# Healthcare-Robotics/mr-gan

Hardware: AMD Instinct MI355X
Metric: GAN train steps/sec (labeled+unlabeled+G) at batch 4096 (higher is better)
Workload: dtype bf16; 1 GPU; BASELINE configs[1]: synthetic N=65536 x D=512, K=6, batch 4096 per GPU, labeled 100/class; one step = D sub-step (3B rows) + G sub-step (2B rows) + both Adam updates; global_batch=4096, rows_per_gpu=4096, parallelism=single, batch_statistics=n/a, launch=hipGraph replay

## Files before the change

include/mrgan_debug.h:

```cpp
#ifndef MRGAN_DEBUG_H
#define MRGAN_DEBUG_H

#include "mrgan_abi.h"

#ifdef __cplusplus
extern "C" {
#endif

int mrgan_debug_noise(mrgan_handle* h, uint32_t site, uint32_t seg, uint32_t step, uint32_t row0, int rows, int cols,
                      float* out_dev, mrgan_stream stream);
int mrgan_debug_tr_probe(uint16_t* out1024_dev, mrgan_stream stream);
int mrgan_debug_ablate(mrgan_handle* h, int bits);
int mrgan_debug_buffer(mrgan_handle* h, int kind, int l, void** ptr_dev, int* rows_per_seg, int* ld, int* elem_size);
int mrgan_debug_gemm_time(int op, int m, int n, int k, int nbatch, int splits, int reps, int ablate, int kc_cfg, float* avg_us);

typedef struct mrgan_debug_gemm_desc {
    int32_t dtype, op, m, n, k, nbatch, splits;
    int32_t kchunk;
    int32_t kc_cfg;
    int32_t tune_bits;
    int32_t seg_stride, seg_rows;
    const void* a; int64_t a_bs, a_si, a_sk;
    const void* b; int64_t b_bs, b_sk, b_sj;
    int32_t act, n_valid;
    const float* bias;
    void* out; int64_t out_bs; int32_t ldo;
    float sigma; uint32_t site, seg0; int32_t seg_step; uint32_t iter_step, row0;
    uint32_t iter;
    uint64_t seed;
    uint16_t* mask; int64_t mask_bs; int32_t ldm;
    const void* h; int64_t h_bs; int32_t ldh;
    int32_t cs_mode; float* cs1; float* cs2; int32_t ldcs;
    const float* bn_mu; const float* bn_rstd;
    float* slab; int64_t slab_stride;
    void* q8; int64_t q8_bs; int32_t ldq8;
    void* q8t; int64_t q8t_bs; int32_t ldq8t;
    const void* slot_a; const void* slot_b; void* slot_o;
    int32_t gauss;
} mrgan_debug_gemm_desc;
typedef struct mrgan_debug_fold { const float* src; float* dst; int64_t stride; int32_t nsrc, n, ngroups; } mrgan_debug_fold;
int mrgan_debug_gemm_launch(const mrgan_debug_gemm_desc* d, int count, int grouped, const mrgan_debug_fold* fold,
                            char* kname, int kname_len, mrgan_stream stream);

int mrgan_debug_gemm_fp8(int m, int n, int k, const float* a_dev, const float* b_dev, const float* bias_dev, int act, float scale_a,
                         float scale_b, float* out_dev, int reps, float* avg_us, int kc_cfg, mrgan_stream stream);

int mrgan_debug_quant8(const void* src, int64_t src_bs, int ld, int rows, int cols, int nb, int prow, void* dst, int64_t dst_bs, int ldd,
                       void* dstt, int64_t dstt_bs, int lddt, void* slot_dev, int fmt, mrgan_stream stream);
int mrgan_debug_fp8_update_scales(void* slots_dev, int n, mrgan_stream stream);

#ifdef __cplusplus
}
#endif
#endif
```

mr_gan_amd/csrc/engine_debug.hip:

```cpp
#include "engine_internal.h"

namespace mrgan {
int launch_tr_probe(unsigned short* out, hipStream_t s);
}

namespace {

template <typename T>
__global__ void to_f32_kernel(const T* src, long lds, float* dst, long ldd, int rows, int cols) {
    const int c = blockIdx.x * 64 + (threadIdx.x & 63), r = blockIdx.y * 4 + (threadIdx.x >> 6);
    if (r >= rows || c >= cols) return;
    dst[(long)r * ldd + c] = Elem<T>::to_f32(src[(long)r * lds + c]);
}

}

extern "C" {

int mrgan_debug_noise(mrgan_handle* h, uint32_t site, uint32_t seg, uint32_t step, uint32_t row0, int rows, int cols, float* out,
                      mrgan_stream stream) {
    if (!h || !out) return fail(-1, "null argument");
    if (h->gauss && (row0 & 1u)) return fail(-1, "debug_noise: a true-Gaussian handle draws row pairs, row0 must be even");
    CHK(launch_noise_debug(h->gauss, h->cfg.seed, site, seg, step, row0, rows, cols, out, (hipStream_t)stream));
    return 0;
}

int mrgan_debug_ablate(mrgan_handle* h, int bits) {
    if (!h) return fail(-1, "null handle");
    if (h->graph_exec) { hipGraphExecDestroy(h->graph_exec); h->graph_exec = nullptr; h->graph_ready = false; }
    h->ablate = bits;
    return 0;
}

int mrgan_debug_buffer(mrgan_handle* h, int kind, int l, void** ptr, int* rows_per_seg, int* ld, int* elem_size) {
    if (!h || !ptr || l < 0 || l > 4) return fail(-1, "debug_buffer: bad argument");
    switch (kind) {
        case 0: *ptr = selected(h, h->xin[l]); *ld = h->d[l].Kp; break;
        case 1: *ptr = selected(h, h->dpre[l]); *ld = h->d[l].Np; break;
        case 2: *ptr = selected(h, h->feat); *ld = h->Fp; break;
        default: return fail(-1, "debug_buffer: unknown kind");
    }
    *rows_per_seg = h->S; *elem_size = h->es;
    return 0;
}

int mrgan_debug_gemm_time(int op, int m, int n, int k, int nbatch, int splits, int reps, int ablate, int kc_cfg, float* avg_us) {
    if ((n % 64) || (k % 64) || !avg_us) return fail(-1, "debug_gemm_time: bad argument");
    const size_t rows = (size_t)m * nbatch;
    const bool is_dx = op == 1 || op >= 5;
    const int a_cols = is_dx ? n : k, o_cols = is_dx ? k : n;
    if (op < 0 || op > 8) return fail(-1, "debug_gemm_time: bad op");
    if (!kc_cfg_supported(kc_cfg)) return fail(-1, "debug_gemm_time: unsupported forward / dX tile config %d", kc_cfg);
    __bf16 *ta = nullptr, *tb = nullptr, *to = nullptr;
    uint16_t* mask = nullptr; float* slabs = nullptr; float* bias = nullptr; DevState* st = nullptr;
    HIPCHK(hipMalloc((void**)&ta, rows * std::max(a_cols, n) * 2));
    HIPCHK(hipMalloc((void**)&tb, (size_t)std::max((size_t)k, rows) * n * 2));
    HIPCHK(hipMalloc((void**)&to, rows * std::max(o_cols, n) * 2));
    HIPCHK(hipMalloc((void**)&mask, (rows / 32 + 4) * std::max(n, k) * 4));
    HIPCHK(hipMalloc((void**)&bias, (size_t)std::max(n, k) * 4));
    HIPCHK(hipMalloc((void**)&st, sizeof(DevState) * 2));
    HIPCHK(hipMemset(ta, 0x3c, rows * std::max(a_cols, n) * 2));
    HIPCHK(hipMemset(tb, 0x3c, (size_t)std::max((size_t)k, rows) * n * 2));
    HIPCHK(hipMemset(mask, 0x55, (rows / 32 + 4) * std::max(n, k) * 4));
    HIPCHK(hipMemset(bias, 0, (size_t)std::max(n, k) * 4));
    HIPCHK(hipMemset(st, 0, sizeof(DevState) * 2));
    GemmArgs g;
    int epi;
    if (op == 0 || op == 3 || op == 4) {
        epi = EPI_FWD; g = gemm_fwd_args(m, k, n, nbatch, ta, (long)m * k, k, tb, k, true);
        g.e.act = ACT_RELU; g.e.n_valid = n; g.e.bias = bias; g.e.ldo = n; g.e.out_bs = (long)m * n;
        g.e.sigma = op == 0 ? 0.5f : 0.f; g.e.site = 1;
        if (op != 4) { g.e.mask = mask; g.e.ldm = n; g.e.mask_bs = (long)(m / 32 + 1) * n * 2; }
    } else if (is_dx) {
        epi = EPI_DX; g = gemm_dx_args(m, k, n, nbatch, ta, (long)m * n, n, tb, n);
        g.e.act = op == 1 ? ACT_RELU : op == 5 ? ACT_SOFTPLUS : ACT_LINEAR; g.e.n_valid = k; g.e.ldo = k; g.e.out_bs = (long)m * k;
        if (op == 1) { g.e.mask = mask; g.e.ldm = k; g.e.mask_bs = (long)(m / 32 + 1) * k * 2; }
        if (op == 5 || op == 6) { g.e.h = ta; g.e.ldh = k; g.e.h_bs = (long)m * k; }
        if (op >= 5 && op <= 7) {
            HIPCHK(hipMalloc((void**)&slabs, (size_t)2 * (rows / 64 + 1) * k * 4));
            g.e.cs_mode = op == 6 ? CS_SUM_XHAT : CS_SUM; g.e.cs1 = slabs; g.e.cs2 = slabs + (size_t)(rows / 64 + 1) * k; g.e.ldcs = k;
            g.e.bn_mu = bias; g.e.bn_rstd = bias;
        }
    } else {
        epi = EPI_SLAB; splits = std::max(1, splits);
        HIPCHK(hipMalloc((void**)&slabs, (size_t)splits * k * n * 4));
        g = gemm_dw_args(k, n, m * nbatch, splits, gemm_dw_kchunk(m * nbatch, splits), 0, 0, ta, k, tb, n, false, slabs);
    }
    g.e.st = st; g.e.out = to; g.e.ablate = ablate; g.e.tune_kc_cfg = kc_cfg; g.e.seed = 1;
#ifdef MRGAN_STAMPS
    unsigned long long* stamps = nullptr;
    if (op != 2) {
        HIPCHK(hipMalloc((void**)&stamps, 4096 * 12 * sizeof(unsigned long long)));
        HIPCHK(hipMemset(stamps, 0, 4096 * 12 * sizeof(unsigned long long)));
        g.e.slab = (float*)stamps;
    }
#endif
    hipEvent_t e0, e1;
    HIPCHK(hipEventCreate(&e0)); HIPCHK(hipEventCreate(&e1));
    int r = 0;
    for (int i = 0; i < 3 && !r; ++i) r = launch_gemm_bf16(epi, g, 0);
    HIPCHK(hipDeviceSynchronize());
    HIPCHK(hipEventRecord(e0, 0));
    for (int i = 0; i < reps && !r; ++i) r = launch_gemm_bf16(epi, g, 0);
    HIPCHK(hipEventRecord(e1, 0));
    HIPCHK(hipEventSynchronize(e1));
    float ms = 0.f;
    HIPCHK(hipEventElapsedTime(&ms, e0, e1));
    *avg_us = 1e3f * ms / (float)reps;
#ifdef MRGAN_STAMPS
    if (stamps) {
        std::vector<unsigned long long> hs(4096 * 12);
        hipMemcpy(hs.data(), stamps, hs.size() * 8, hipMemcpyDeviceToHost);
        double tot[10] = {0, 0, 0, 0, 0, 0, 0, 0, 0, 0}; int nb = 0;
        for (int b = 0; b < 4096; ++b) if (hs[b * 12 + 2]) { ++nb; for (int i = 0; i < 10; ++i) tot[i] += (double)hs[b * 12 + i]; }
        if (nb) fprintf(stderr, "  stamps (kcycles per block, %d blocks): setup %.1f | fill %.1f | mainloop %.1f | barrier %.1f | epilogue %.1f (math+staging %.1f, barrier %.1f, copy-out %.1f, column sums %.1f) | tail-barrier %.1f\n",
                        nb, tot[0] / nb / 1e3, tot[1] / nb / 1e3, tot[2] / nb / 1e3, tot[3] / nb / 1e3, tot[4] / nb / 1e3, tot[6] / nb / 1e3, tot[7] / nb / 1e3, tot[8] / nb / 1e3,
                        tot[9] / nb / 1e3, tot[5] / nb / 1e3);
        hipFree(stamps);
    }
#endif
    hipEventDestroy(e0); hipEventDestroy(e1);
    hipFree(ta); hipFree(tb); hipFree(to); hipFree(mask); hipFree(bias); hipFree(st);
    if (slabs) hipFree(slabs);
    if (r) return fail(r, "debug_gemm_time: launch failed (%d)", r);
    return 0;
}

int mrgan_debug_gemm_fp8(int m, int n, int k, const float* a, const float* b, const float* bias, int act, float scale_a, float scale_b,
                         float* out, int reps, float* avg_us, int kc_cfg, mrgan_stream stream) {
    if ((n % 64) || (k % 128) || !a || !b) return fail(-1, "debug_gemm_fp8: n %% 64 == 0 and k %% 128 == 0 are required");
    hipStream_t s = (hipStream_t)stream;
    unsigned char *ta = nullptr, *tb = nullptr;
    __bf16* to = nullptr;
    HIPCHK(hipMalloc((void**)&ta, (size_t)m * k));
    HIPCHK(hipMalloc((void**)&tb, (size_t)n * k));
    HIPCHK(hipMalloc((void**)&to, (size_t)m * n * 2));
    CHK(launch_to_fp8(a, k, ta, k, m, k, m, k, scale_a, 0, s));
    CHK(launch_to_fp8(b, n, tb, k, k, n, k, n, scale_b, 1, s));
    GemmArgs g = gemm_fwd_args(m, k, n, 1, ta, 0, k, tb, k, true);
    g.e.act = act; g.e.n_valid = n; g.e.bias = bias; g.e.out = to; g.e.ldo = n; g.e.acc_scale = 1.0f / (scale_a * scale_b);
    g.e.tune_kc_cfg = kc_cfg;
#ifdef MRGAN_STAMPS
    unsigned long long* stamps = nullptr;
    HIPCHK(hipMalloc((void**)&stamps, 4096 * 4 * sizeof(unsigned long long)));
    g.e.cs2 = (float*)stamps;
#endif
    int r = launch_gemm_fp8(EPI_FWD, g, s);
#ifdef MRGAN_STAMPS
    HIPCHK(hipMemsetAsync(stamps, 0, 4096 * 4 * sizeof(unsigned long long), s));
#endif
    if (!r && reps > 0 && avg_us) {
        hipEvent_t e0, e1;
        HIPCHK(hipEventCreate(&e0)); HIPCHK(hipEventCreate(&e1));
        HIPCHK(hipStreamSynchronize(s));
        HIPCHK(hipEventRecord(e0, s));
        for (int i = 0; i < reps && !r; ++i) r = launch_gemm_fp8(EPI_FWD, g, s);
        HIPCHK(hipEventRecord(e1, s));
        HIPCHK(hipEventSynchronize(e1));
        float ms = 0.f;
        HIPCHK(hipEventElapsedTime(&ms, e0, e1));
        *avg_us = 1e3f * ms / (float)reps;
        hipEventDestroy(e0); hipEventDestroy(e1);
    }
    if (!r && out) hipLaunchKernelGGL(to_f32_kernel<__bf16>, grid2d(m, n), dim3(256), 0, s, (const __bf16*)to, (long)n, out, (long)n, m, n);
    hipStreamSynchronize(s);
#ifdef MRGAN_STAMPS
    {
        std::vector<unsigned long long> hs(4096 * 4);
        hipMemcpy(hs.data(), stamps, hs.size() * 8, hipMemcpyDeviceToHost);
        double cyc = 0, wait = 0, rt = 0, tiles = 0; int nb = 0;
        for (int b = 0; b < 4096; ++b) if (hs[b * 4 + 3]) { cyc += hs[b * 4]; wait += hs[b * 4 + 1]; rt += hs[b * 4 + 2]; tiles += hs[b * 4 + 3]; ++nb; }
        if (nb) fprintf(stderr, "[stamps] fp8 %dx%dx%d: blocks %d, tiles/block %.1f, k-loop cycles/tile %.0f (wait+barrier %.0f = %.1f %%), per k-tile %.0f, clock %.3f GHz\n",
                        m, n, k, nb, tiles / nb, cyc / tiles, wait / tiles, 100.0 * wait / cyc, cyc / tiles / (k / 128), cyc / rt * 0.1);
        hipFree(stamps);
    }
#endif
    hipFree(ta); hipFree(tb); hipFree(to);
    if (r) return fail(r, "debug_gemm_fp8: launch failed (%d)", r);
    return 0;
}

int mrgan_debug_tr_probe(uint16_t* out, mrgan_stream stream) {
    if (!out) return fail(-1, "null argument");
    CHK(launch_tr_probe(out, (hipStream_t)stream));
    return 0;
}

static int debug_gemm_args(const mrgan_debug_gemm_desc& d, const DevState* st, GemmArgs& g, int& epi) {
    const bool bf = d.dtype == MRGAN_BF16, f8 = d.dtype == MRGAN_FP8;
    if (!bf && !f8 && d.dtype != MRGAN_F32) return fail(-1, "debug_gemm_launch: dtype must be fp32, bf16 or fp8");
    if (d.op < 0 || d.op > 2) return fail(-1, "debug_gemm_launch: op must be 0, 1 or 2");
    if (!kc_cfg_supported(d.kc_cfg)) return fail(-1, "debug_gemm_launch: kc_cfg %d is not a block tile", d.kc_cfg);
    if (d.m < 1 || d.n < 1 || d.k < 1 || d.nbatch < 1 || d.splits < 1 || !d.a || !d.b) return fail(-1, "debug_gemm_launch: empty problem");
    if (d.n % 64) return fail(-1, "debug_gemm_launch: n must be a multiple of 64");
    epi = d.op == 0 ? EPI_FWD : d.op == 1 ? EPI_DX : EPI_SLAB;
    if (epi == EPI_FWD) g = gemm_fwd_args(d.m, d.k, d.n, d.nbatch, d.a, d.a_bs, d.a_si, d.b, d.b_sj, true);
    else if (epi == EPI_DX) g = gemm_dx_args(d.m, d.n, d.k, d.nbatch, d.a, d.a_bs, d.a_si, d.b, d.b_sj);
    else if (f8) g = gemm_dw_args(d.m, d.n, d.k, 1, d.k, 0, 0, d.a, d.a_si, d.b, d.b_sj, true, d.slab);
    else g = gemm_dw_args(d.m, d.n, d.k, 1, d.k, 0, 0, d.a, d.a_sk, d.b, d.b_sk, false, d.slab);
    g.nbatch = d.nbatch; g.splits = d.splits;
    if (d.kchunk > 0) g.kchunk = d.kchunk;
    if (d.seg_stride > 0) { g.seg_stride = d.seg_stride; g.seg_rows = d.seg_rows; }
    g.a_bs = d.a_bs; g.a_si = d.a_si; g.a_sk = d.a_sk;
    g.b_bs = d.b_bs; g.b_sk = d.b_sk; g.b_sj = d.b_sj;
    Epi& e = g.e;
    e.act = d.act; e.n_valid = d.n_valid; e.bias = d.bias;
    e.out = d.out; e.out_bs = d.out_bs; e.ldo = d.ldo;
    e.sigma = d.sigma; e.site = d.site; e.seg0 = d.seg0; e.seg_step = d.seg_step; e.iter_step = d.iter_step; e.row0 = d.row0; e.seed = d.seed;
    e.mask = d.mask; e.mask_bs = d.mask_bs; e.ldm = d.ldm;
    e.h = d.h; e.h_bs = d.h_bs; e.ldh = d.ldh;
    e.cs_mode = d.cs_mode; e.cs1 = d.cs1; e.cs2 = d.cs2; e.ldcs = d.ldcs; e.bn_mu = d.bn_mu; e.bn_rstd = d.bn_rstd;
    e.slab = d.slab; e.slab_stride = d.slab_stride;
    e.st = st; e.acc_scale = 1.f; e.tune_kc_cfg = d.kc_cfg; e.tune_bits = d.tune_bits;
    e.gauss = d.gauss;
    if (f8) {
        e.q8 = d.q8; e.q8_bs = d.q8_bs; e.ldq8 = d.ldq8; e.q8t = d.q8t; e.q8t_bs = d.q8t_bs; e.ldq8t = d.ldq8t;
        e.qa = (const Fp8Slot*)d.slot_a; e.qb = (const Fp8Slot*)d.slot_b; e.qo = (Fp8Slot*)d.slot_o;
        if (epi == EPI_SLAB ? d.ldo < d.n : (d.out && (d.ldo < d.n || (d.ldo % 8)))) return fail(-1, "debug_gemm_launch: fp8 product needs ldo >= n (bf16: a multiple of 8)");
        if ((d.a_si % 16) || (d.b_sj % 16) || (d.a_bs % 16) || (d.b_bs % 16)) return fail(-1, "debug_gemm_launch: fp8 row and batch pitches must be multiples of 16 bytes");
        if (d.q8 && (d.q8_bs % 16)) return fail(-1, "debug_gemm_launch: q8_bs must be a multiple of 16");
        if (d.q8 && d.ldq8 < d.n) return fail(-1, "debug_gemm_launch: ldq8 >= n");
        if (d.q8t && (d.q8t_bs < 0 || d.ldq8t < (d.nbatch - 1) * d.q8t_bs + round_up(d.m, 16))) return fail(-1, "debug_gemm_launch: ldq8t must hold nbatch batches of round_up(m, 16) bytes");
    }
    if (epi == EPI_SLAB && !f8) {
        const int bk = bf ? 64 : 16;
        if (!d.slab || d.ldo < d.n) return fail(-1, "debug_gemm_launch: weight gradient needs slab and ldo >= n");
        if ((g.kchunk % bk) || (g.seg_stride % bk)) return fail(-1, "debug_gemm_launch: kchunk and seg_stride must be multiples of %d", bk);
        if (bf && ((d.a_sk % 8) || (d.b_sk % 8) || d.a_sk < round_up(d.m, 8))) return fail(-1, "debug_gemm_launch: bf16 row pitches must be multiples of 8");
    } else if (epi != EPI_SLAB) {
        if ((!f8 && !d.out) || (d.out && d.ldo < d.n) || d.n_valid < 0 || d.n_valid > d.n) return fail(-1, "debug_gemm_launch: needs out, ldo >= n and n_valid <= n");
        if (bf && ((d.ldo % 8) || (d.a_si % 8) || (d.b_sj % 8))) return fail(-1, "debug_gemm_launch: bf16 row pitches must be multiples of 8");
        if (d.cs_mode != CS_NONE && (!d.cs1 || d.ldcs < d.n || (d.cs_mode != CS_SUM && !d.cs2))) return fail(-1, "debug_gemm_launch: column sums need cs1 / cs2 and ldcs >= n");
        if (d.cs_mode == CS_SUM_XHAT && (epi != EPI_DX || !d.bn_mu || !d.bn_rstd || !d.h)) return fail(-1, "debug_gemm_launch: xhat sums need bn_mu, bn_rstd and h on a dX product");
        if (epi == EPI_DX && d.act == ACT_SOFTPLUS && !d.h) return fail(-1, "debug_gemm_launch: the softplus derivative needs h");
        if (epi == EPI_DX && d.act == ACT_RELU && !d.mask) return fail(-1, "debug_gemm_launch: the relu derivative needs mask");
        if (d.h && (d.ldh < d.n || (bf && (d.ldh % 8)))) return fail(-1, "debug_gemm_launch: ldh");
        if (d.mask && d.ldm < d.n) return fail(-1, "debug_gemm_launch: ldm >= n");
    }
    return 0;
}

int mrgan_debug_gemm_launch(const mrgan_debug_gemm_desc* d, int count, int grouped, const mrgan_debug_fold* fold,
                            char* kname, int kname_len, mrgan_stream stream) {
    if (!d || count < 1) return fail(-1, "null argument");
    if (kname && kname_len > 0) kname[0] = 0;
    hipStream_t s = (hipStream_t)stream;
    DevState* st = nullptr;
    DevState hst[2];
    memset(hst, 0, sizeof hst);
    hst[0].iter = hst[1].iter = d[0].iter;
    HIPCHK(hipMalloc((void**)&st, sizeof hst));
    hipError_t he = hipMemcpy(st, hst, sizeof hst, hipMemcpyHostToDevice);
    const char* name = "";
    int r = he == hipSuccess ? 0 : fail(-10, "hipMemcpy failed: %s", hipGetErrorString(he));
    if (!r && !grouped) {
        GemmArgs g;
        int epi = 0;
        if (count != 1) r = fail(-1, "debug_gemm_launch: one product per plain launch");
        if (!r) r = debug_gemm_args(d[0], st, g, epi);
        if (!r) {
            r = d[0].dtype == MRGAN_FP8    ? launch_gemm_fp8(epi, g, s, &name)
                : d[0].dtype == MRGAN_BF16 ? launch_gemm_bf16(epi, g, s, &name)
                                           : launch_gemm_f32(epi, g, s, &name);
            if (r) fail(r, "debug_gemm_launch: launch refused (%d)", r);
        }
    } else if (!r) {
        GemmArgs gs[KS_GROUP_MAX];
        for (int i = 0; i < count && i < KS_GROUP_MAX && !r; ++i) {
            int epi = 0;
            r = debug_gemm_args(d[i], st, gs[i], epi);
            if (!r && (epi != EPI_SLAB || d[i].dtype != MRGAN_BF16)) r = fail(-1, "debug_gemm_launch: grouped launches are bf16 weight gradients");
        }
        FoldJob fj;
        memset(&fj, 0, sizeof fj);
        if (!r && fold) {
            if (!fold->src || !fold->dst || fold->nsrc < 1 || fold->n < 1 || fold->ngroups < 1 || fold->stride < fold->n)
                r = fail(-1, "debug_gemm_launch: fold");
            fj.src = fold->src; fj.dst = fold->dst; fj.stride = fold->stride; fj.nsrc = fold->nsrc; fj.n = fold->n; fj.ngroups = fold->ngroups;
        }
        if (!r) {
            r = launch_gemm_bf16_dw_group(gs, count, s, &name, fold ? &fj : nullptr);
            if (r < 0) fail(r, "debug_gemm_launch: grouped launch failed (%d)", r);
        }
    }
    he = hipStreamSynchronize(s);
    hipFree(st);
    if (!r && he != hipSuccess) return fail(-10, "debug_gemm_launch: %s", hipGetErrorString(he));
    if (!r && kname && kname_len > 0) snprintf(kname, (size_t)kname_len, "%s", name);
    return r;
}

int mrgan_debug_quant8(const void* src, int64_t src_bs, int ld, int rows, int cols, int nb, int prow, void* dst, int64_t dst_bs, int ldd,
                       void* dstt, int64_t dstt_bs, int lddt, void* slot, int fmt, mrgan_stream stream) {
    if (!src || rows < 0 || rows > prow || cols < 1 || cols > ld || (fmt != FP8_E4M3 && fmt != FP8_E5M2)) return fail(-1, "debug_quant8: bad argument");
    if ((dst && ldd < cols) || (dstt && (dstt_bs < 0 || lddt < (int64_t)(nb - 1) * dstt_bs + prow))) return fail(-1, "debug_quant8: ldd >= cols, lddt >= nb batches of prow bytes");
    Quant8Args a;
    memset(&a, 0, sizeof a);
    a.src = (const __bf16*)src; a.src_bs = src_bs; a.ld = ld; a.rows = rows; a.cols = cols; a.nb = nb; a.prow = prow;
    a.dst = (unsigned char*)dst; a.dst_bs = dst_bs; a.ldd = ldd;
    a.dstt = (unsigned char*)dstt; a.dstt_bs = dstt_bs; a.lddt = lddt;
    a.slot = (Fp8Slot*)slot; a.fmt = fmt;
    hipStream_t s = (hipStream_t)stream;
    const int r = launch_quant8(a, s);
    if (r) return fail(r, "debug_quant8: launch refused (%d)", r);
    HIPCHK(hipStreamSynchronize(s));
    return 0;
}

int mrgan_debug_fp8_update_scales(void* slots, int n, mrgan_stream stream) {
    if (!slots || n < 1) return fail(-1, "debug_fp8_update_scales: bad argument");
    hipStream_t s = (hipStream_t)stream;
    CHK(launch_fp8_update_scales((Fp8Slot*)slots, n, s));
    HIPCHK(hipStreamSynchronize(s));
    return 0;
}

}
```

mr_gan_amd/csrc/gemm.h:

```cpp
#pragma once
#include <string.h>

#include <algorithm>

#include "common.h"

namespace mrgan {

enum { EPI_FWD = 0, EPI_DX = 1, EPI_SLAB = 2 };
enum { VAR_ACT_MASK = 3, VAR_NOISE = 4, VAR_MASK = 8, VAR_GAUSS = 16, VAR_DYN = 64 };


struct Epi {
    int act;
    int n_valid;
    const float* bias;
    void* out; long out_bs; int ldo;
    float sigma; uint32_t site; uint32_t seg0;
    int seg_step; uint32_t iter_step;
    uint32_t row0;
    uint64_t seed;
    int gauss;
    uint16_t* mask; long mask_bs; int ldm;
    const void* h; long h_bs; int ldh;
    int cs_mode; float* cs1; float* cs2; int ldcs;
    const float* bn_mu; const float* bn_rstd;
    float* slab; long slab_stride;
    const DevState* st;
    int ablate;
    float acc_scale;
    const Fp8Slot* qa; const Fp8Slot* qb;
    Fp8Slot* qo;
    void* q8; long q8_bs; int ldq8;
    void* q8t; long q8t_bs; int ldq8t;
    int tune_kc_cfg;
    int tune_bits;
    long model_stride;
    int segs;
    uint32_t model_mul;
};

struct GemmArgs {
    int M, N, K;
    int nbatch, splits;
    int kchunk;
    int tiles_m;
    int seg_stride, seg_rows;
    const void* A; long a_bs, a_si, a_sk;
    const void* B; long b_bs, b_sk, b_sj;
    Epi e;
};

__device__ __forceinline__ int batch_model(const Epi& e, int batch) { return (int)(((uint32_t)batch * e.model_mul) >> 16); }
__device__ __forceinline__ int batch_segment(const Epi& e, int batch, int model) { return batch - model * e.segs; }
template <typename P>
__device__ __forceinline__ P* model_ptr(P* p, const Epi& e, int model) { return (P*)((char*)p + (long)model * e.model_stride); }
template <typename P>
__device__ __forceinline__ const P* model_ptr(const P* p, const Epi& e, int model) { return (const P*)((const char*)p + (long)model * e.model_stride); }

__device__ __forceinline__ uint32_t relu_mask_bit(const uint16_t* mask, int ldm, int row, int col) {
    const int rr = row & 31;
    const uint32_t w = mask[((long)(row >> 5) * ldm + col) * 2 + ((rr >> 2) & 1)];
    return (w >> ((rr & 3) | ((rr >> 3) << 2))) & 1u;
}

template <int MR, int NR>
struct EpiPrefetch {
    float bias[NR];
    float mu[NR], rstd[NR];
    uint32_t mbits[MR][NR];
    uint32_t iter;
};

template <int VAR>
__device__ __host__ __forceinline__ bool dx_needs_h(const Epi& e) {
    if constexpr ((VAR & VAR_DYN) != 0) return e.h && (e.act == ACT_SOFTPLUS || e.cs_mode == CS_SUM_XHAT);
    else if constexpr ((VAR & VAR_ACT_MASK) == ACT_SOFTPLUS) return true;
    else if constexpr ((VAR & VAR_ACT_MASK) == ACT_LINEAR) return e.cs_mode == CS_SUM_XHAT;
    else return false;
}

template <typename T, int EPI, int MR, int NR, int VAR>
__device__ __forceinline__ void epilogue_prefetch(EpiPrefetch<MR, NR>& pf, const GemmArgs& g, int batch , int model,
                                                  int row_blk, int col_blk, int wm, int wn, int lane) {
    const Epi& e = g.e;
    const int lc = lane & 31, lh = lane >> 5;
    const int act = (VAR & 64) ? e.act : (VAR & 3);
    pf.iter = 0u;
    if constexpr (EPI == EPI_FWD && ((VAR & VAR_DYN) || (VAR & VAR_NOISE))) { if (e.st) pf.iter = e.st->iter; }
#pragma unroll
    for (int ni = 0; ni < NR; ++ni) {
        const int col = col_blk + (wn * NR + ni) * 32 + lc;
        pf.bias[ni] = 0.f; pf.mu[ni] = 0.f; pf.rstd[ni] = 0.f;
        if constexpr (EPI == EPI_FWD) { if (col < e.n_valid && e.bias) pf.bias[ni] = model_ptr(e.bias, e, model)[col]; }
        if constexpr (EPI == EPI_DX) {
            if (e.cs_mode == CS_SUM_XHAT) {
                const bool cok = col < e.n_valid && col < g.N;
                const int cc = cok ? col : 0;
                const float m = e.bn_mu[cc], r = e.bn_rstd[cc];
                pf.mu[ni] = cok ? m : 0.f; pf.rstd[ni] = cok ? r : 0.f;
            }
        }
#pragma unroll
        for (int mi = 0; mi < MR; ++mi) {
            pf.mbits[mi][ni] = 0;
            if constexpr (EPI == EPI_DX) {
                const int rsub = row_blk + (wm * MR + mi) * 32;
                if (act == ACT_RELU && e.mask && col < g.N && rsub < g.M)
                    pf.mbits[mi][ni] = (model_ptr(e.mask, e, model) + (long)batch * e.mask_bs)[((long)(rsub >> 5) * e.ldm + col) * 2 + lh];
            }
        }
    }
}

template <typename T, int EPI, int MR, int NR, int WM, bool STAGED = false, int VAR = VAR_DYN, int Q8 = -1>
__device__ __forceinline__ void epilogue(f32x16 (&acc)[MR][NR], const GemmArgs& g, int batch , int model, int split,
                                         int tile_m, int row_blk, int col_blk, int wm, int wn, int lane,
                                         float* lds ,
                                         int bn , T* tile = nullptr,
                                         const EpiPrefetch<MR, NR>* pf = nullptr,
                                         const T* htile = nullptr ,
                                         unsigned long long* est = nullptr ) {
#ifdef MRGAN_STAMPS
#define EPI_STAMP(i) do { if (est) { const unsigned long long n_ = __builtin_amdgcn_s_memtime(); est[i] += n_ - est[4]; est[4] = n_; } } while (0)
    if (est) est[4] = __builtin_amdgcn_s_memtime();
#else
#define EPI_STAMP(i)
#endif
    const Epi& e = g.e;
    const int lc = lane & 31, lh = lane >> 5;
    const int M = g.M;
    if (e.ablate & 2) { if (acc[0][0][0] == 12345.678f) ((float*)e.out)[0] = 1.f; return; }

    if constexpr (EPI == EPI_SLAB) {
        float* dst = model_ptr(e.slab, e, model) + (long)(batch * g.splits + split) * e.slab_stride;
#pragma unroll
        for (int mi = 0; mi < MR; ++mi)
#pragma unroll
            for (int ni = 0; ni < NR; ++ni) {
                const int col = col_blk + (wn * NR + ni) * 32 + lc;
#pragma unroll
                for (int r = 0; r < 16; ++r) {
                    const int row = row_blk + (wm * MR + mi) * 32 + acc_row(r, lh);
                    if (row < M && col < g.N) dst[(long)row * e.ldo + col] = acc[mi][ni][r];
                }
            }
        return;
    } else {
        constexpr bool DYN = (VAR & VAR_DYN) != 0;
        const int act = DYN ? e.act : (VAR & VAR_ACT_MASK);
        constexpr bool fast_math = sizeof(T) == 2;
        T* out = (T*)model_ptr(e.out, e, model) + (long)batch * e.out_bs;
        constexpr bool MASKED = !DYN && (EPI == EPI_DX || (VAR & VAR_MASK));
        uint16_t* mask = nullptr;
        if constexpr (MASKED) mask = model_ptr(e.mask, e, model) + (long)batch * e.mask_bs;
        else if (DYN && e.mask) mask = model_ptr(e.mask, e, model) + (long)batch * e.mask_bs;
        const T* hprev = e.h ? (const T*)model_ptr(e.h, e, model) + (long)batch * e.h_bs : nullptr;
        float* const cs1p = model_ptr(e.cs1, e, model);
        float* const cs2p = model_ptr(e.cs2, e, model);
        const bool noisy = EPI == EPI_FWD && (DYN ? e.sigma > 0.f : (VAR & VAR_NOISE) != 0);
        constexpr bool GAUSS = (VAR & VAR_GAUSS) != 0;
        uint32_t rowhash[MR];
        i32x4 hfrag = {0, 0, 0, 0};
        const float sigs = GAUSS ? e.sigma : e.sigma * NOISE_SCALE;
        if constexpr (EPI == EPI_FWD) {
            if (noisy) {
                const uint32_t nkey = noise_key(e.seed + (uint64_t)model, e.site * 256u + e.seg0 + (uint32_t)(batch * e.seg_step),
                                                (pf ? pf->iter : (e.st ? e.st->iter : 0u)) + (uint32_t)batch * e.iter_step);
                if constexpr (!GAUSS) hfrag = hadamard_frag(lane);
#pragma unroll
                for (int mi = 0; mi < MR; ++mi) {
                    if constexpr (GAUSS) rowhash[mi] = gauss_pairhash(nkey, e.row0 + (uint32_t)(row_blk + (wm * MR + mi) * 32), lane);
                    else rowhash[mi] = noise_rowhash(nkey, e.row0 + (uint32_t)(row_blk + (wm * MR + mi) * 32 + lc));
                }
            }
        }

        float q8_scale = 1.f, q8_amax = 0.f;
        float q8_cs[MR][NR];
        if constexpr (Q8 >= 0) {
            q8_scale = e.qo->scale;
#pragma unroll
            for (int mi = 0; mi < MR; ++mi)
#pragma unroll
                for (int ni = 0; ni < NR; ++ni) q8_cs[mi][ni] = 0.f;
        }
        float keep[MR][NR][16];
#pragma unroll
        for (int ni = 0; ni < NR; ++ni) {
            const int col = col_blk + (wn * NR + ni) * 32 + lc;
            const bool colvalid = col < e.n_valid;
            const bool colin = col < g.N;
            float bias = 0.f;
            if constexpr (EPI == EPI_FWD) {
                if (pf) bias = pf->bias[ni];
                else if (colvalid && e.bias) bias = model_ptr(e.bias, e, model)[col];
            }
            const float sig = (noisy && colvalid) ? sigs : 0.f;
#pragma unroll
            for (int mi = 0; mi < MR; ++mi) {
                const int rsub = row_blk + (wm * MR + mi) * 32;
                const long mword = ((long)(rsub >> 5) * e.ldm + col) * 2 + lh;
                uint32_t mbits = 0;
                if constexpr (EPI == EPI_DX) {
                    if (pf) mbits = pf->mbits[mi][ni];
                    else if (act == ACT_RELU && colin && rsub < M) mbits = mask[mword];
                }
                i32x16 nzs = {0, 0, 0, 0, 0, 0, 0, 0, 0, 0, 0, 0, 0, 0, 0, 0};
                f32x16 nzg = {0.f, 0.f, 0.f, 0.f, 0.f, 0.f, 0.f, 0.f, 0.f, 0.f, 0.f, 0.f, 0.f, 0.f, 0.f, 0.f};
                if constexpr (EPI == EPI_FWD) {
                    if constexpr (GAUSS) { if (noisy) nzg = gauss_block(rowhash[mi], (uint32_t)col, lane); }
                    else if (noisy) nzs = noise_block(rowhash[mi], (uint32_t)col >> 5, lane, hfrag);
                }
#pragma unroll
                for (int q = 0; q < 4; ++q) {
                    const int r4 = rsub + 4 * lh + 8 * q;
                    float o4[4];
#pragma unroll
                    for (int j = 0; j < 4; ++j) {
                        const int r = 4 * q + j, row = r4 + j;
                        float v = acc[mi][ni][r];
                        float& o = o4[j];
                        if constexpr (EPI == EPI_FWD) {
                            v += bias;
                            if (act == ACT_RELU) {
                                v = fmaxf(v, 0.f);
                                if (MASKED || mask) mbits |= min(__builtin_bit_cast(uint32_t, v), 1u) << r;
                            } else if (act == ACT_SOFTPLUS) {
                                v = colvalid ? (fast_math ? softplus_fast(v) : softplus_f(v)) : 0.f;
                            }
                            if constexpr (GAUSS) o = noisy ? fmaf(sig, nzg[r], v) : v;
                            else o = noisy ? fmaf(sig, (float)nzs[r], v) : v;
                        } else {
                            if (act == ACT_RELU)
                                v = __builtin_bit_cast(float, __builtin_bit_cast(uint32_t, v) & (uint32_t)(-(int)((mbits >> r) & 1u)));
                            else if (act == ACT_SOFTPLUS) {
                                float hv;
                                if (STAGED && htile) hv = (row < M && colin) ? Elem<T>::to_f32(htile[(row - row_blk) * bn + (col - col_blk)]) : 0.f;
                                else hv = (row < M && colin) ? Elem<T>::to_f32(hprev[(long)row * e.ldh + col]) : 0.f;
                                v *= fast_math ? one_minus_exp_neg_fast(hv) : -expm1f(-hv);
                            }
                            o = v;
                        }
                        if constexpr (Q8 < 0) keep[mi][ni][r] = v;
                        if constexpr (!STAGED) { if (row < M && colin) out[(long)row * e.ldo + col] = Elem<T>::from_f32(o); }
                    }
                    if constexpr (Q8 >= 0) {
                        constexpr int BMT = WM * MR * 32;
                        if (rsub + 32 > M) {
#pragma unroll
                            for (int j = 0; j < 4; ++j) o4[j] = (r4 + j < M) ? o4[j] : 0.f;
                        }
                        q8_amax = fmaxf(q8_amax, fmaxf(fmaxf(fabsf(o4[0]), fabsf(o4[1])), fmaxf(fabsf(o4[2]), fabsf(o4[3]))));
                        if constexpr (EPI == EPI_DX) q8_cs[mi][ni] += (o4[0] + o4[1]) + (o4[2] + o4[3]);
                        const uint32_t w = fp8_pack4<Q8>(o4[0], o4[1], o4[2], o4[3], q8_scale);
                        unsigned char* q8r = (unsigned char*)tile;
                        unsigned char* q8c = q8r + BMT * (bn + 16);
                        const int rl = r4 - row_blk, cl = col - col_blk;
                        *(uint32_t*)(q8c + cl * (BMT + 16) + rl) = w;
                        const int kq = lane & 3;
                        *(uint32_t*)(q8r + (rl + kq) * (bn + 16) + (cl - kq)) = quad_byte_transpose(w);
                    } else if constexpr (STAGED) {
                        T* tp = tile + (r4 - row_blk) * bn + (col - col_blk);
                        if constexpr (sizeof(T) == 2) {
                            typedef __attribute__((ext_vector_type(2))) __bf16 bf16x2_t;
                            typedef __attribute__((ext_vector_type(2))) float f32x2_t;
                            const bf16x2_t p01 = __builtin_convertvector((f32x2_t){o4[0], o4[1]}, bf16x2_t);
                            const bf16x2_t p23 = __builtin_convertvector((f32x2_t){o4[2], o4[3]}, bf16x2_t);
                            tp[0] = p01[0]; tp[bn] = p01[1]; tp[2 * bn] = p23[0]; tp[3 * bn] = p23[1];
                        } else {
#pragma unroll
                            for (int j = 0; j < 4; ++j) tp[j * bn] = Elem<T>::from_f32(o4[j]);
                        }
                    }
                }
                if constexpr (EPI == EPI_FWD) {
                    if (act == ACT_RELU && (MASKED || mask) && colin && rsub < M) mask[mword] = (uint16_t)mbits;
                }
            }
        }

        EPI_STAMP(0);
        if constexpr (Q8 >= 0) {
            fp8_amax_commit(e.qo, q8_amax);
        } else if constexpr (STAGED) {
            typedef __attribute__((ext_vector_type(4))) unsigned int u32x4_t;
            constexpr int EPV = 16 / (int)sizeof(T);
            const int chunks_per_row = bn / EPV, bm = WM * MR * 32;
            __syncthreads();
            EPI_STAMP(1);
            for (int cidx = threadIdx.x; cidx < bm * chunks_per_row; cidx += blockDim.x) {
                const int r = cidx / chunks_per_row, c = cidx - r * chunks_per_row;
                if (e.out && row_blk + r < M && col_blk + c * EPV < g.N)
                    *(u32x4_t*)(out + (long)(row_blk + r) * e.ldo + col_blk + c * EPV) = *(const u32x4_t*)(tile + r * bn + c * EPV);
            }
            EPI_STAMP(2);
        }

        if constexpr (Q8 >= 0) {
            static_assert(MR >= 2 && (MR % 2) == 0, "Q8 epilogue: each wave covers whole 64-row groups");
            if (EPI == EPI_DX && e.cs_mode == CS_SUM) {
                const long prow0 = (long)batch * g.tiles_m + (row_blk >> 6);
#pragma unroll
                for (int hh = 0; hh < MR / 2; ++hh)
#pragma unroll
                    for (int ni = 0; ni < NR; ++ni) {
                        float s1 = q8_cs[2 * hh][ni] + q8_cs[2 * hh + 1][ni];
                        s1 += __shfl_xor(s1, 32, 64);
                        const int col = col_blk + (wn * NR + ni) * 32 + lc;
                        const long pr = prow0 + wm * (MR / 2) + hh;
                        if (lh == 0 && col < g.N && col < e.ldcs && row_blk + (wm * (MR / 2) + hh) * 64 < M) cs1p[pr * e.ldcs + col] = s1;
                    }
            }
        } else if (e.cs_mode != CS_NONE) {
            constexpr int NH = MR >= 2 ? MR / 2 : 1, MH = MR >= 2 ? 2 : 1;
            float cs1[NH][NR], cs2[NH][NR];
#pragma unroll
            for (int hh = 0; hh < NH; ++hh)
#pragma unroll
                for (int ni = 0; ni < NR; ++ni) {
                    const int col = col_blk + (wn * NR + ni) * 32 + lc;
                    float s1 = 0.f, s2 = 0.f;
#pragma unroll
                    for (int m2 = 0; m2 < MH; ++m2) {
                        const int mi = hh * MH + m2;
                        const int rsub = row_blk + (wm * MR + mi) * 32 + 4 * lh;
                        if (e.cs_mode == CS_SUM_XHAT) {
                            const bool cok = col < e.n_valid && col < g.N;
                            const float mu = pf ? pf->mu[ni] : (cok ? e.bn_mu[col] : 0.f), rstd = pf ? pf->rstd[ni] : (cok ? e.bn_rstd[col] : 0.f);
#pragma unroll
                            for (int r = 0; r < 16; ++r) {
                                const int row = rsub + (r & 3) + 8 * (r >> 2);
                                const bool ok = row < M;
                                const float v = ok ? keep[mi][ni][r] : 0.f;
                                float hv;
                                if (STAGED && htile) hv = (ok && cok) ? Elem<T>::to_f32(htile[(row - row_blk) * bn + (col - col_blk)]) : mu;
                                else hv = (ok && cok) ? Elem<T>::to_f32(hprev[(long)row * e.ldh + col]) : mu;
                                s1 += v; s2 = fmaf(v * (hv - mu), rstd, s2);
                            }
                        } else {
#pragma unroll
                            for (int r = 0; r < 16; ++r) {
                                const float v = (rsub + (r & 3) + 8 * (r >> 2) < M) ? keep[mi][ni][r] : 0.f;
                                s1 += v; s2 = fmaf(v, v, s2);
                            }
                        }
                    }
                    cs1[hh][ni] = s1 + __shfl_xor(s1, 32, 64);
                    cs2[hh][ni] = s2 + __shfl_xor(s2, 32, 64);
                }
            const long prow0 = (long)batch * g.tiles_m + (row_blk >> 6);
            if constexpr (MR >= 2) {
                if (lh == 0) {
#pragma unroll
                    for (int hh = 0; hh < NH; ++hh)
#pragma unroll
                        for (int ni = 0; ni < NR; ++ni) {
                            const int col = col_blk + (wn * NR + ni) * 32 + lc;
                            const long pr = prow0 + wm * NH + hh;
                            if (col < g.N && col < e.ldcs && row_blk + (wm * NH + hh) * 64 < M) {
                                cs1p[pr * e.ldcs + col] = cs1[hh][ni];
                                if (e.cs_mode != CS_SUM) cs2p[pr * e.ldcs + col] = cs2[hh][ni];
                            }
                        }
                }
            } else {
                const int wcols = NR * 32;
                __syncthreads();
                if (lh == 0) {
#pragma unroll
                    for (int ni = 0; ni < NR; ++ni) {
                        const int c = wn * wcols + ni * 32 + lc;
                        lds[(wm * 2 + 0) * bn + c] = cs1[0][ni];
                        lds[(wm * 2 + 1) * bn + c] = cs2[0][ni];
                    }
                }
                __syncthreads();
                const int t = threadIdx.x;
                if (t < bn) {
                    float s1 = 0.f, s2 = 0.f;
#pragma unroll
                    for (int w = 0; w < WM; ++w) { s1 += lds[(w * 2 + 0) * bn + t]; s2 += lds[(w * 2 + 1) * bn + t]; }
                    if (col_blk + t < g.N && col_blk + t < e.ldcs) {
                        cs1p[prow0 * e.ldcs + col_blk + t] = s1;
                        if (e.cs_mode != CS_SUM) cs2p[prow0 * e.ldcs + col_blk + t] = s2;
                    }
                }
            }
        }
        EPI_STAMP(3);
    }
#undef EPI_STAMP
}

enum { TUNE_BIT_NO_KS_GROUP = 4 };
inline bool kc_cfg_supported(int cfg) {
    return cfg == -1 || cfg == 0 || cfg == 1 || cfg == 3 || cfg == 5 || cfg == 7 || cfg == 9;
}
constexpr int KS_GROUP_MAX = 6;
struct FoldJob { const float* src; float* dst; long stride; int nsrc, n, ngroups, blocks_x; long model_stride; };
struct KsGroup {
    int n;
    int blk_end[KS_GROUP_MAX];
    FoldJob fold;
    GemmArgs g[KS_GROUP_MAX];
};

int launch_gemm_f32(int epi, const GemmArgs& g, hipStream_t s, const char** kname = nullptr);
int launch_gemm_bf16(int epi, const GemmArgs& g, hipStream_t s, const char** kname = nullptr);
int launch_gemm_fp8(int epi, const GemmArgs& g, hipStream_t s, const char** kname = nullptr);
int launch_to_fp8(const float* src, long ld_src, unsigned char* dst, long ld_dst, int rows, int cols, int prow, int pcol, float scale,
                  int transpose, hipStream_t s);
struct Quant8Args {
    const __bf16* src; long src_bs; int ld; int rows, cols, nb;
    int prow;
    unsigned char* dst; long dst_bs; int ldd;
    unsigned char* dstt; long dstt_bs; int lddt;
    Fp8Slot* slot; int fmt;
};
int launch_quant8(const Quant8Args& a, hipStream_t s);
int launch_fp8_update_scales(Fp8Slot* slots, int n, hipStream_t s);
int launch_fp8_init_slots(Fp8Slot* slots, int n, const float* targets_dev, hipStream_t s);
int launch_gemm_bf16_dw_group(const GemmArgs* gs, int n, hipStream_t s, const char** kname = nullptr,
                              const FoldJob* fold = nullptr);

constexpr int GEMM_NO_HOLES = 1 << 30;
inline GemmArgs gemm_args(int M, int N, int K, int nbatch, int tile_rows) {
    GemmArgs g;
    memset(&g, 0, sizeof g);
    g.M = M; g.N = N; g.K = K; g.nbatch = nbatch; g.splits = 1; g.kchunk = K; g.tiles_m = ceil_div(M, tile_rows);
    g.seg_stride = g.seg_rows = GEMM_NO_HOLES;
    return g;
}
inline GemmArgs gemm_fwd_args(int rows, int K, int N, int nb, const void* x, long a_bs, long lda, const void* w, long ldw,
                              bool w_transposed) {
    GemmArgs g = gemm_args(rows, N, K, nb, 64);
    g.A = x; g.a_bs = a_bs; g.a_si = lda; g.a_sk = 1;
    g.B = w;
    if (w_transposed) { g.b_sj = ldw; g.b_sk = 1; }
    else { g.b_sk = ldw; g.b_sj = 1; }
    return g;
}
inline GemmArgs gemm_dx_args(int rows, int K, int N, int nb, const void* dy, long a_bs, long ldy, const void* w, long ldw) {
    GemmArgs g = gemm_args(rows, K, N, nb, 64);
    g.A = dy; g.a_bs = a_bs; g.a_si = ldy; g.a_sk = 1;
    g.B = w; g.b_sk = 1; g.b_sj = ldw;
    return g;
}
inline int gemm_dw_kchunk(int vrows, int splits) { return (int)round_up(ceil_div(vrows, splits), 64); }
inline GemmArgs gemm_dw_args(int K, int N, int vrows, int splits, int kchunk, int seg_stride, int seg_rows, const void* x, long ldx,
                             const void* dy, long ldy, bool transposed, float* slab) {
    GemmArgs g = gemm_args(K, N, vrows, 1, 128);
    g.splits = splits; g.kchunk = kchunk;
    if (seg_stride > 0) { g.seg_stride = seg_stride; g.seg_rows = seg_rows; }
    g.A = x; g.B = dy;
    if (transposed) { g.a_si = ldx; g.a_sk = 1; g.b_sj = ldy; g.b_sk = 1; }
    else { g.a_si = 1; g.a_sk = ldx; g.b_sk = ldy; g.b_sj = 1; }
    g.e.slab = slab; g.e.slab_stride = (long)K * N; g.e.ldo = N;
    return g;
}
inline GemmArgs gemm_group(GemmArgs g, int models, long model_stride) {
    if (models <= 1) return g;
    g.e.segs = g.nbatch; g.e.model_stride = model_stride;
    g.e.model_mul = (65536u + (uint32_t)g.nbatch - 1) / (uint32_t)g.nbatch + ((65536u % (uint32_t)g.nbatch) == 0 ? 1u : 0u);
    g.nbatch *= models;
    return g;
}
inline int gemm_model_batches(const GemmArgs& g) { return g.e.segs > 0 ? g.e.segs : g.nbatch; }
inline int gemm_models(const GemmArgs& g) { return g.e.segs > 0 ? g.nbatch / g.e.segs : 1; }
inline long mask_pitch(int seg_rows, int ldm) { return (long)(seg_rows / 32) * ldm * 2; }

inline int epi_variant(int epi, const Epi& e) {
    if (e.act != ACT_LINEAR && e.act != ACT_RELU && e.act != ACT_SOFTPLUS) return -1;
    if (epi != EPI_FWD) return e.act;
    const bool noise = e.sigma > 0.f, mask = e.mask != nullptr;
    if (e.act == ACT_RELU ? (noise && !mask) : (mask || (noise && e.act == ACT_SOFTPLUS))) return -1;
    return e.act | (noise ? VAR_NOISE : 0) | (mask ? VAR_MASK : 0) | (noise && e.gauss ? VAR_GAUSS : 0);
}
inline int persistent_grid(int tiles, int lds_bytes) { return std::min(tiles, 256 * std::max(1, (160 * 1024) / lds_bytes)); }
template <auto KERN, int LDS, typename... Args>
int launch_with_dyn_lds(dim3 grid, dim3 block, hipStream_t s, const Args&... args) {
    static_assert(LDS <= 160 * 1024, "LDS budget of a CU");
    static DeviceOnce attr;
    if (attr.first()) {
        if (hipFuncSetAttribute((const void*)KERN, hipFuncAttributeMaxDynamicSharedMemorySize, LDS) != hipSuccess) return -2;
        attr.mark();
    }
    MRGAN_LAUNCH(KERN, grid, block, LDS, s, args...);
    return 0;
}

}
```

mr_gan_amd/csrc/gemm_bf16.hip:

```cpp
#include <algorithm>
#include <cstring>
#include <string>

#include "gemm.h"
#include "lds_ring.h"

namespace mrgan {

namespace {
constexpr int BN = 128, BK = RING_BK;
constexpr int KS_PITCH = 320;
constexpr int KS_TILE_BYTES = 64 * KS_PITCH;

#ifdef MRGAN_STAMPS
struct KcStamps { unsigned long long acc[6], prev, epi[5]; };
#define KC_STAMPS_PARAM , KcStamps& stamps_
#define KC_STAMPS_ARG , stamps_
#else
#define KC_STAMPS_PARAM
#define KC_STAMPS_ARG
#endif
template <int EPI, int BM, int BNT, int WM, int WN, int NS, int VAR>
__device__ __forceinline__ void kc_tile(const GemmArgs& g, const int batch , const int model, const int tile_m, const int tile_n, char* lds KC_STAMPS_PARAM) {
    constexpr int NW = WM * WN;
    constexpr int MR = BM / WM / 32, NR = BNT / WN / 32;
    constexpr int A_BYTES = BM * 128, B_BYTES = BNT * 128, STAGE = A_BYTES + B_BYTES;
    constexpr int A_INSTR = BM / 8 / NW, B_INSTR = BNT / 8 / NW;
    static_assert(MR >= 1 && NR >= 1 && A_INSTR >= 1 && B_INSTR >= 1 && BM % (8 * NW) == 0 && BNT % (8 * NW) == 0, "tile/wave layout");
    const int t = threadIdx.x, lane = t & 63;
    const int wave = __builtin_amdgcn_readfirstlane(t >> 6);
    const int wm = wave / WN, wn = wave % WN;
    const int lrow = lane >> 3, lp = lane & 7;
    const int lr = lane & 31, lh = lane >> 5;
    const int nk = (g.e.ablate & 4) ? 0 : g.K / BK;
#ifdef MRGAN_STAMPS
#define STAMP(i) do { const unsigned long long n_ = __builtin_amdgcn_s_memtime(); stamps_.acc[i] += n_ - stamps_.prev; stamps_.prev = n_; } while (0)
#else
#define STAMP(i)
#endif
    {
        const int row_blk = tile_m * BM, col_blk = tile_n * BNT;

        const __bf16* Ab = model_ptr((const __bf16*)g.A, g.e, model) + (long)batch * g.a_bs;
        const __bf16* Bb = model_ptr((const __bf16*)g.B, g.e, model) + (long)batch * g.b_bs;
        const __amdgpu_buffer_rsrc_t rsA = __builtin_amdgcn_make_buffer_rsrc((void*)Ab, 0, (int)((long)g.M * g.a_si * 2), 0x00020000);
        const __amdgpu_buffer_rsrc_t rsB = __builtin_amdgcn_make_buffer_rsrc((void*)Bb, 0, (int)((long)g.N * g.b_sj * 2), 0x00020000);
        int voffA[A_INSTR], voffB[B_INSTR];
#pragma unroll
        for (int i = 0; i < A_INSTR; ++i) {
            const int R = (wave * A_INSTR + i) * 8 + lrow;
            voffA[i] = (int)(((long)(row_blk + R) * g.a_si + ((lp ^ ((R >> 1) & 7)) << 3)) * 2);
        }
#pragma unroll
        for (int i = 0; i < B_INSTR; ++i) {
            const int R = (wave * B_INSTR + i) * 8 + lrow;
            voffB[i] = (int)(((long)(col_blk + R) * g.b_sj + ((lp ^ ((R >> 1) & 7)) << 3)) * 2);
        }
        auto issue = [&](int k0, int buf) {
            char* a_dst = lds + buf * STAGE + wave * A_INSTR * 1024;
            char* b_dst = lds + buf * STAGE + A_BYTES + wave * B_INSTR * 1024;
#pragma unroll
            for (int i = 0; i < A_INSTR; ++i) glds16(rsA, a_dst + i * 1024, voffA[i], k0 * 2);
#pragma unroll
            for (int i = 0; i < B_INSTR; ++i) glds16(rsB, b_dst + i * 1024, voffB[i], k0 * 2);
        };

#pragma unroll
        for (int p = 0; p < NS - 1; ++p)
            if (p < nk) issue(p * BK, p);


        const __bf16* htile = nullptr;
        if constexpr (EPI == EPI_DX && (VAR & VAR_ACT_MASK) != ACT_RELU) {
            if (dx_needs_h<VAR>(g.e)) {
                constexpr int OUTB = BM * BNT * 2 + 4 * WM * BNT * 4, RING = NS * STAGE;
                char* hdst = lds + (RING > OUTB ? RING : OUTB);
                const __bf16* hb = model_ptr((const __bf16*)g.e.h, g.e, model) + (long)batch * g.e.h_bs;
                const __amdgpu_buffer_rsrc_t rsH = __builtin_amdgcn_make_buffer_rsrc((void*)hb, 0, (int)((long)g.M * g.e.ldh * 2), 0x00020000);
                constexpr int RPI = 1024 / (BNT * 2);
                constexpr int LPR = 64 / RPI;
                constexpr int HI = BM / RPI / NW;
#pragma unroll
                for (int i = 0; i < HI; ++i) {
                    const int R = (wave * HI + i) * RPI + lane / LPR;
                    const int voff = (int)(((long)(row_blk + R) * g.e.ldh + col_blk) * 2) + (lane % LPR) * 16;
                    glds16(rsH, hdst + (wave * HI + i) * 1024, voff, 0);
                }
                htile = (const __bf16*)hdst;
            }
        }

        f32x16 acc[MR][NR];
#pragma unroll
        for (int i = 0; i < MR; ++i)
#pragma unroll
            for (int j = 0; j < NR; ++j)
#pragma unroll
                for (int r = 0; r < 16; ++r) acc[i][j][r] = 0.f;

        EpiPrefetch<MR, NR> pf;
        epilogue_prefetch<__bf16, EPI, MR, NR, VAR>(pf, g, batch, model, row_blk, col_blk, wm, wn, lane);

#define KC_FRAG_A(As, mi, ks) *(const bf16x8*)(As + kc_off((wm * MR + mi) * 32 + lr, (ks) * 2 + lh))
#define KC_FRAG_B(Bs, ni, ks) *(const bf16x8*)(Bs + kc_off((wn * NR + ni) * 32 + lr, (ks) * 2 + lh))
        RING_MAINLOOP(NS, A_INSTR + B_INSTR, MR, NR, nk, acc, issue, 0, KC_FRAG_A, KC_FRAG_B, lds, STAGE, A_BYTES, STAMP)
#undef KC_FRAG_A
#undef KC_FRAG_B
        STAMP(2);
        __syncthreads();
        STAMP(3);
        epilogue<__bf16, EPI, MR, NR, WM, true, VAR>(acc, g, batch, model, 0, tile_m, row_blk, col_blk, wm, wn, lane,
                                                     (float*)(lds + BM * BNT * 2), BNT, (__bf16*)lds, &pf, htile
#ifdef MRGAN_STAMPS
                                                     , stamps_.epi
#endif
                                                     );
        STAMP(4);
        __syncthreads();
        STAMP(5);
    }
#undef STAMP
}

template <int EPI, int BM, int BNT, int WM, int WN, int NS, int VAR>
__global__ __launch_bounds__(64 * WM * WN) void gemm_bf16_kc_kernel(const GemmArgs g) {
    extern __shared__ __attribute__((aligned(16))) char lds[];
    const int ntn = (g.N + BNT - 1) / BNT, ntm = (g.M + BM - 1) / BM;
    const int ntiles = ntn * ntm * g.nbatch;
#ifdef MRGAN_STAMPS
    KcStamps stamps_ = {{0, 0, 0, 0, 0, 0}, __builtin_amdgcn_s_memtime(), {0, 0, 0, 0, 0}};
#endif
    for (int tl = blockIdx.x; tl < ntiles; tl += gridDim.x) {
        const int tidx = xcd_tile(tl, ntiles);
        const int bidx = tidx / (ntn * ntm), rem = tidx - bidx * (ntn * ntm);
        const int model = batch_model(g.e, bidx), batch = batch_segment(g.e, bidx, model);
        int tile_m, tile_n;
        if ((ntm & 3) == 0 && ntn >= 8 && g.K >= 2048) {
            const int grp = rem / (4 * ntn), in = rem - grp * (4 * ntn);
            tile_m = grp * 4 + (in & 3); tile_n = in >> 2;
        } else { tile_m = rem / ntn; tile_n = rem - tile_m * ntn; }
        kc_tile<EPI, BM, BNT, WM, WN, NS, VAR>(g, batch, model, tile_m, tile_n, lds KC_STAMPS_ARG);
    }
#ifdef MRGAN_STAMPS
    if (g.e.slab && threadIdx.x == 0)
    {
        for (int i = 0; i < 6; ++i) ((unsigned long long*)g.e.slab)[(long)blockIdx.x * 12 + i] = stamps_.acc[i];
        for (int i = 0; i < 4; ++i) ((unsigned long long*)g.e.slab)[(long)blockIdx.x * 12 + 6 + i] = stamps_.epi[i];
    }
#endif
}

thread_local const char* g_last_kernel = "";

template <int EPI, int BM, int BNT, int WM, int WN, int NS, int VAR>
int launch_kc(const GemmArgs& g, hipStream_t s) {
    static const std::string name = "gemm_bf16_kc_kernel<" + std::to_string(EPI) + ", " + std::to_string(BM) + ", " +
                                    std::to_string(BNT) + ", " + std::to_string(WM) + ", " + std::to_string(WN) + ", " +
                                    std::to_string(NS) + ", " + std::to_string(VAR) + ">";
    g_last_kernel = name.c_str();
    constexpr int STAGE = BM * 128 + BNT * 128;
    constexpr int OUT = BM * BNT * 2 + 4 * WM * BNT * 4;
    constexpr int LDS = (NS * STAGE > OUT ? NS * STAGE : OUT) + ((EPI == EPI_DX && (VAR & VAR_ACT_MASK) != ACT_RELU) ? BM * BNT * 2 : 0);
    const int tiles = ceil_div(g.M, BM) * ceil_div(g.N, BNT) * g.nbatch;
    return launch_with_dyn_lds<gemm_bf16_kc_kernel<EPI, BM, BNT, WM, WN, NS, VAR>, LDS>(dim3(persistent_grid(tiles, LDS)), dim3(64 * WM * WN), s, g);
}

__device__ __forceinline__ bf16x8 ks_frag_swz(const char* tile, int fb, int ks, int lane) {
    const int g4 = lane >> 4, i16 = lane & 15, q = i16 >> 2, p = i16 & 3;
    const int f0 = fb + (g4 & 1) * 16;
    const int m0 = ks * 16 + (g4 >> 1) * 8;
    const char* a0 = tile + (m0 + q) * 256 + ((((f0 >> 3) + (p >> 1)) ^ (q << 2)) << 4) + ((p & 1) << 3);
    const s16x4 t0 = __builtin_amdgcn_ds_read_tr16_b64_v4i16((lds_s16x4*)a0);
    const s16x4 t1 = __builtin_amdgcn_ds_read_tr16_b64_v4i16((lds_s16x4*)(a0 + 4 * 256));
    const s16x8 tt = __builtin_shufflevector(t0, t1, 0, 1, 2, 3, 4, 5, 6, 7);
    return __builtin_bit_cast(bf16x8, tt);
}

template <int NS, int WM, int WN>
__device__ __forceinline__ void ks_fast_body(const GemmArgs& g, const int bid, const int model ) {
    constexpr int NW = WM * WN;
    constexpr int MR = 128 / WM / 32, NR = 128 / WN / 32;
    constexpr int T_BYTES = 64 * 256, STAGE = 2 * T_BYTES;
    constexpr int T_INSTR = 16 / NW;
    static_assert(MR >= 1 && NR >= 1 && T_INSTR >= 1, "tile/wave layout");
    extern __shared__ __attribute__((aligned(16))) char lds[];

    const int t = threadIdx.x, lane = t & 63;
    const int wave = __builtin_amdgcn_readfirstlane(t >> 6);
    const int wm = wave / WN, wn = wave % WN;
    const int ntn = (g.N + 127) / 128, ntm = (g.M + 127) / 128;
    const int tidx = xcd_tile(bid, ntn * ntm * g.splits);
    const int split = tidx / (ntn * ntm), rem = tidx - split * (ntn * ntm);
    int tile_m, tile_n;
    if ((ntm & 7) == 0 && ntn >= 16) {
        const int grp = rem / (8 * ntn), in = rem - grp * (8 * ntn);
        tile_m = grp * 8 + (in & 7); tile_n = in >> 3;
    } else { tile_m = rem / ntn; tile_n = rem - tile_m * ntn; }
    const int row_blk = tile_m * 128, col_blk = tile_n * 128;
    const int k_begin = split * g.kchunk;
    const int k_end = (g.e.ablate & 4) ? k_begin : min(g.K, k_begin + g.kchunk);

    const __amdgpu_buffer_rsrc_t rsA = __builtin_amdgcn_make_buffer_rsrc((void*)model_ptr(g.A, g.e, model), 0, (int)((long)g.K * g.a_sk * 2), 0x00020000);
    const __amdgpu_buffer_rsrc_t rsB = __builtin_amdgcn_make_buffer_rsrc((void*)model_ptr(g.B, g.e, model), 0, (int)((long)g.K * g.b_sk * 2), 0x00020000);
    const int lrow = lane >> 4, lp = lane & 15;
    int voffA[T_INSTR], voffB[T_INSTR];
#pragma unroll
    for (int i = 0; i < T_INSTR; ++i) {
        const int kr = (wave * T_INSTR + i) * 4 + lrow;
        const int c = lp ^ ((kr & 3) << 2);
        voffA[i] = (int)(((long)kr * g.a_sk + row_blk + c * 8) * 2);
        voffB[i] = (int)(((long)kr * g.b_sk + col_blk + c * 8) * 2);
    }
    auto issue = [&](int k0, int buf) {
        char* a_dst = lds + buf * STAGE + wave * T_INSTR * 1024;
        char* b_dst = a_dst + T_BYTES;
#pragma unroll
        for (int i = 0; i < T_INSTR; ++i) glds16(rsA, a_dst + i * 1024, voffA[i], (int)((long)k0 * g.a_sk * 2));
#pragma unroll
        for (int i = 0; i < T_INSTR; ++i) glds16(rsB, b_dst + i * 1024, voffB[i], (int)((long)k0 * g.b_sk * 2));
    };

    f32x16 acc[MR][NR];
#pragma unroll
    for (int i = 0; i < MR; ++i)
#pragma unroll
        for (int j = 0; j < NR; ++j)
#pragma unroll
            for (int r = 0; r < 16; ++r) acc[i][j][r] = 0.f;

    const int nk = (k_end - k_begin + BK - 1) / BK;
#pragma unroll
    for (int p = 0; p < NS - 1; ++p)
        if (p < nk) issue(k_begin + p * BK, p);
#define KS_FRAG_A(As, mi, ks) ks_frag_swz(As, (wm * MR + mi) * 32, ks, lane)
#define KS_FRAG_B(Bs, ni, ks) ks_frag_swz(Bs, (wn * NR + ni) * 32, ks, lane)
#define KS_NO_STAMP(i)
    RING_MAINLOOP(NS, 2 * T_INSTR, MR, NR, nk, acc, issue, k_begin, KS_FRAG_A, KS_FRAG_B, lds, STAGE, T_BYTES, KS_NO_STAMP)
#undef KS_FRAG_A
#undef KS_FRAG_B
#undef KS_NO_STAMP
    __syncthreads();
    epilogue<__bf16, EPI_SLAB, MR, NR, WM>(acc, g, 0, model, split, tile_m, row_blk, col_blk, wm, wn, lane, (float*)lds, BN);
}

template <int NS, int WM, int WN>
__global__ __launch_bounds__(64 * WM * WN) void gemm_bf16_ks_fast_kernel(const GemmArgs g) {
    ks_fast_body<NS, WM, WN>(g, blockIdx.x, blockIdx.y);
}

template <int NS, int WM, int WN>
__global__ __launch_bounds__(64 * WM * WN) void gemm_bf16_ks_group_kernel(const KsGroup grp) {
    const int ngemm = grp.blk_end[grp.n - 1];
    if ((int)blockIdx.x >= ngemm) {
        const FoldJob& f = grp.fold;
        const float* fsrc = (const float*)((const char*)f.src + (long)blockIdx.y * f.model_stride);
        float* fdst = (float*)((char*)f.dst + (long)blockIdx.y * f.model_stride);
        const int fb = (int)blockIdx.x - ngemm, gidx = fb / f.blocks_x;
        const int i = (fb - gidx * f.blocks_x) * 256 + (int)threadIdx.x;
        if (threadIdx.x >= 256 || i >= f.n) return;
        float s0 = 0.f, s1 = 0.f, s2 = 0.f, s3 = 0.f;
        int p = gidx;
        for (; p + 3 * f.ngroups < f.nsrc; p += 4 * f.ngroups) {
            s0 += fsrc[(long)p * f.stride + i]; s1 += fsrc[(long)(p + f.ngroups) * f.stride + i];
            s2 += fsrc[(long)(p + 2 * f.ngroups) * f.stride + i]; s3 += fsrc[(long)(p + 3 * f.ngroups) * f.stride + i];
        }
        for (; p < f.nsrc; p += f.ngroups) s0 += fsrc[(long)p * f.stride + i];
        fdst[(long)gidx * f.stride + i] = (s0 + s1) + (s2 + s3);
        return;
    }
    int i = 0, b0 = 0;
#pragma unroll
    for (int j = 0; j < KS_GROUP_MAX - 1; ++j)
        if (j + 1 < grp.n && (int)blockIdx.x >= grp.blk_end[j]) { i = j + 1; b0 = grp.blk_end[j]; }
    ks_fast_body<NS, WM, WN>(grp.g[i], (int)blockIdx.x - b0, blockIdx.y);
}

template <int NS, int WM, int WN>
int launch_ks_fast(const GemmArgs& g, hipStream_t s) {
    static const std::string name = "gemm_bf16_ks_fast_kernel<" + std::to_string(NS) + ", " + std::to_string(WM) + ", " + std::to_string(WN) + ">";
    g_last_kernel = name.c_str();
    constexpr int STAGE = 2 * 64 * 256;
    dim3 grid(ceil_div(g.N, 128) * ceil_div(g.M, 128) * g.splits, gemm_models(g));
    return launch_with_dyn_lds<gemm_bf16_ks_fast_kernel<NS, WM, WN>, NS * STAGE>(grid, dim3(64 * WM * WN), s, g);
}

__device__ __forceinline__ bf16x8 ks_frag(const char* tile, int fb, int ks, int lane) {
    const int g4 = lane >> 4, i16 = lane & 15, q = i16 >> 2, p = i16 & 3;
    const int f0 = fb + (g4 & 1) * 16;
    const int m0 = ks * 16 + (g4 >> 1) * 8;
    const char* a0 = tile + (m0 + q) * KS_PITCH + (f0 + 4 * p) * 2;
    const s16x4 t0 = __builtin_amdgcn_ds_read_tr16_b64_v4i16((lds_s16x4*)a0);
    const s16x4 t1 = __builtin_amdgcn_ds_read_tr16_b64_v4i16((lds_s16x4*)(a0 + 4 * KS_PITCH));
    const s16x8 tt = __builtin_shufflevector(t0, t1, 0, 1, 2, 3, 4, 5, 6, 7);
    return __builtin_bit_cast(bf16x8, tt);
}

__global__ __launch_bounds__(256) void gemm_bf16_ks_kernel(const GemmArgs g) {
    __shared__ __attribute__((aligned(16))) char lds[2 * KS_TILE_BYTES];
    char* As = lds;
    char* Bs = lds + KS_TILE_BYTES;

    const int t = threadIdx.x, lane = t & 63, wave = t >> 6;
    const int wm = wave >> 1, wn = wave & 1;
    const int tile_n = blockIdx.x, tile_m = blockIdx.y;
    const int bidx = blockIdx.z / g.splits, split = blockIdx.z % g.splits;
    const int model = batch_model(g.e, bidx), batch = batch_segment(g.e, bidx, model);
    const int row_blk = tile_m * 128, col_blk = tile_n * BN;
    const int k_begin = split * g.kchunk;
    const int k_end = (g.e.ablate & 4) ? k_begin : min(g.K, k_begin + g.kchunk);

    const __bf16* A = model_ptr((const __bf16*)g.A, g.e, model) + (long)batch * g.a_bs;
    const __bf16* B = model_ptr((const __bf16*)g.B, g.e, model) + (long)batch * g.b_bs;

    f32x16 acc[2][2];
#pragma unroll
    for (int i = 0; i < 2; ++i)
#pragma unroll
        for (int j = 0; j < 2; ++j)
#pragma unroll
            for (int r = 0; r < 16; ++r) acc[i][j][r] = 0.f;

    u32x4 ra[4], rb[4];
    auto load_tile = [&](int k0) {
        const int kloc = k0 % g.seg_stride;
#pragma unroll
        for (int u = 0; u < 4; ++u) {
            const int cidx = t + 256 * u, kr = cidx >> 4, c = cidx & 15;
            const u32x4 z = {0u, 0u, 0u, 0u};
            const bool kok = (k0 + kr) < k_end && (kloc + kr) < g.seg_rows;
            ra[u] = (kok && row_blk + c * 8 < g.M) ? *(const u32x4*)(A + (long)(k0 + kr) * g.a_sk + row_blk + c * 8) : z;
            rb[u] = (kok && col_blk + c * 8 < g.N) ? *(const u32x4*)(B + (long)(k0 + kr) * g.b_sk + col_blk + c * 8) : z;
        }
    };
    auto store_tile = [&]() {
#pragma unroll
        for (int u = 0; u < 4; ++u) {
            const int cidx = t + 256 * u, kr = cidx >> 4, c = cidx & 15;
            *(u32x4*)(As + kr * KS_PITCH + c * 16) = ra[u];
            *(u32x4*)(Bs + kr * KS_PITCH + c * 16) = rb[u];
        }
    };

    if (k_begin < k_end) {
        load_tile(k_begin);
        for (int k0 = k_begin; k0 < k_end; k0 += BK) {
            __syncthreads();
            store_tile();
            __syncthreads();
            if (k0 + BK < k_end) load_tile(k0 + BK);
#pragma unroll
            for (int ks = 0; ks < BK / 16; ++ks) {
                bf16x8 a[2], b[2];
#pragma unroll
                for (int mi = 0; mi < 2; ++mi) a[mi] = ks_frag(As, (wm * 2 + mi) * 32, ks, lane);
#pragma unroll
                for (int ni = 0; ni < 2; ++ni) b[ni] = ks_frag(Bs, (wn * 2 + ni) * 32, ks, lane);
#pragma unroll
                for (int mi = 0; mi < 2; ++mi)
#pragma unroll
                    for (int ni = 0; ni < 2; ++ni)
                        acc[mi][ni] = __builtin_amdgcn_mfma_f32_32x32x16_bf16(a[mi], b[ni], acc[mi][ni], 0, 0, 0);
            }
        }
    }
    __syncthreads();
    epilogue<__bf16, EPI_SLAB, 2, 2, 2>(acc, g, batch, model, split, tile_m, row_blk, col_blk, wm, wn, lane, (float*)lds, BN);
}

__global__ void tr_probe_kernel(unsigned short* out) {
    __shared__ __attribute__((aligned(16))) unsigned short img[16 * 160];
    const int l = threadIdx.x;
    for (int i = l; i < 16 * 160; i += 64) img[i] = (unsigned short)i;
    __syncthreads();
    const s16x4 t = __builtin_amdgcn_ds_read_tr16_b64_v4i16((lds_s16x4*)((const char*)img + l * 8));
    for (int j = 0; j < 4; ++j) out[l * 8 + j] = (unsigned short)t[j];
    for (int j = 4; j < 8; ++j) out[l * 8 + j] = 0;
    __syncthreads();
    for (int i = l; i < 16 * 160; i += 64) img[i] = (unsigned short)(((i / 160) << 8) | (i % 160));
    __syncthreads();
    const s16x8 f = __builtin_bit_cast(s16x8, ks_frag((const char*)img, 0, 0, l));
    for (int j = 0; j < 8; ++j) out[512 + l * 8 + j] = (unsigned short)f[j];
}
}

template <int EPI, int VAR>
static int launch_kc_tile(const GemmArgs& g, hipStream_t s) {
    int cfg = g.e.tune_kc_cfg;
    if (cfg < 0) {
        const int nbm = gemm_model_batches(g);
        const int t128 = ceil_div(g.M, 128) * ceil_div(g.N, 128) * nbm;
        const int t256 = ceil_div(g.M, 256) * ceil_div(g.N, 256) * nbm;
        cfg = t128 >= 384 ? 7 : 0;
        if (g.K >= 2048 && t256 >= 256 && (g.N % 256) == 0) cfg = 3;
        if (EPI == EPI_FWD && cfg == 7 && g.K >= 1024 && g.K < 2048 && g.N <= 512) cfg = 5;
        if (EPI == EPI_FWD && cfg == 0 && g.K >= 1024 && g.K < 2048 && t128 >= 256 && (g.N % 128) == 0) cfg = 7;
        if (cfg == 0 && ceil_div(g.M, 64) * ceil_div(g.N, 128) * nbm <= 256) cfg = 9;
    }
    if (cfg >= 2 && cfg != 9 && (g.N % 128) != 0) cfg = 0;
    if (cfg == 3 && (g.N % 256) != 0) cfg = 1;
    constexpr bool H_TILE = EPI == EPI_DX && (VAR & VAR_ACT_MASK) != ACT_RELU;
    if (H_TILE && cfg >= 2 && cfg != 9) cfg = 1;
    if constexpr (!H_TILE) {
        if (cfg == 7) return launch_kc<EPI, 128, 128, 2, 4, 2, VAR>(g, s);
        if (cfg == 3) return launch_kc<EPI, 256, 256, 2, 4, 2, VAR>(g, s);
    }
    if (cfg == 9) return launch_kc<EPI, 64, 64, 2, 2, 3, VAR>(g, s);
    if (cfg == 1) return launch_kc<EPI, 128, 128, 2, 2, 2, VAR>(g, s);
    if (cfg == 5) return launch_kc<EPI, 64, 128, 2, 2, 2, VAR>(g, s);
    return launch_kc<EPI, 64, 128, 2, 2, 3, VAR>(g, s);
}

static int launch_kc_any(int epi, const GemmArgs& g, hipStream_t s) {
    const int var = epi_variant(epi, g.e);
    if (epi == EPI_FWD) {
        switch (var) {
            case ACT_RELU | VAR_NOISE | VAR_MASK | VAR_GAUSS: return launch_kc_tile<EPI_FWD, ACT_RELU | VAR_NOISE | VAR_MASK | VAR_GAUSS>(g, s);
            case ACT_LINEAR | VAR_NOISE | VAR_GAUSS: return launch_kc_tile<EPI_FWD, ACT_LINEAR | VAR_NOISE | VAR_GAUSS>(g, s);
            case ACT_RELU | VAR_NOISE | VAR_MASK: return launch_kc_tile<EPI_FWD, ACT_RELU | VAR_NOISE | VAR_MASK>(g, s);
            case ACT_RELU | VAR_MASK: return launch_kc_tile<EPI_FWD, ACT_RELU | VAR_MASK>(g, s);
            case ACT_RELU: return launch_kc_tile<EPI_FWD, ACT_RELU>(g, s);
            case ACT_LINEAR | VAR_NOISE: return launch_kc_tile<EPI_FWD, ACT_LINEAR | VAR_NOISE>(g, s);
            case ACT_LINEAR: return launch_kc_tile<EPI_FWD, ACT_LINEAR>(g, s);
            case ACT_SOFTPLUS: return launch_kc_tile<EPI_FWD, ACT_SOFTPLUS>(g, s);
            default: return -3;
        }
    }
    switch (var) {
        case ACT_RELU: return launch_kc_tile<EPI_DX, ACT_RELU>(g, s);
        case ACT_SOFTPLUS: return launch_kc_tile<EPI_DX, ACT_SOFTPLUS>(g, s);
        default: return launch_kc_tile<EPI_DX, ACT_LINEAR>(g, s);
    }
}

static bool ks_dense_k(const GemmArgs& g) {
    return g.a_si == 1 && g.b_sj == 1 && gemm_model_batches(g) == 1 && (g.K % BK) == 0 && (g.kchunk % BK) == 0 &&
           (g.seg_rows >= g.seg_stride || g.K <= g.seg_rows) &&
           (long)g.K * g.a_sk * 2 < (1L << 31) && (long)g.K * g.b_sk * 2 < (1L << 31);
}

int launch_gemm_bf16_dw_group(const GemmArgs* gs, int n, hipStream_t s, const char** kname, const FoldJob* fold) {
    if (n < 1 || n > KS_GROUP_MAX) return 1;
    if (gs[0].e.tune_bits & TUNE_BIT_NO_KS_GROUP) return 1;
    KsGroup grp;
    memset(&grp, 0, sizeof grp);
    grp.n = n;
    int total = 0;
    const int models = gemm_models(gs[0]);
    for (int i = 0; i < n; ++i) {
        if (!ks_dense_k(gs[i]) || gemm_models(gs[i]) != models) return 1;
        const int blocks = ceil_div(gs[i].N, 128) * ceil_div(gs[i].M, 128) * gs[i].splits;
        total += blocks;
        grp.blk_end[i] = total;
        grp.g[i] = gs[i];
    }
    if (fold && fold->n > 0) {
        grp.fold = *fold;
        grp.fold.blocks_x = ceil_div(fold->n, 256);
        total += grp.fold.blocks_x * fold->ngroups;
    }
    constexpr int STAGE = 2 * 64 * 256, LDS = 2 * STAGE;
    if (const int r = launch_with_dyn_lds<gemm_bf16_ks_group_kernel<2, 2, 4>, LDS>(dim3(total, models), dim3(512), s, grp)) return r;
    if (kname) *kname = "gemm_bf16_ks_group_kernel<2, 2, 4>";
    return hipGetLastError() == hipSuccess ? 0 : -2;
}

int launch_gemm_bf16(int epi, const GemmArgs& g, hipStream_t s, const char** kname) {
    int r = 0;
    if (epi == EPI_SLAB) {
        if (g.a_si != 1 || g.b_sj != 1) return -3;
        if (ks_dense_k(g)) {
            r = launch_ks_fast<3, 2, 4>(g, s);
        } else {
            dim3 grid(ceil_div(g.N, BN), ceil_div(g.M, 128), g.nbatch * g.splits);
            MRGAN_LAUNCH(gemm_bf16_ks_kernel, grid, dim3(256), 0, s, g);
            g_last_kernel = "gemm_bf16_ks_kernel";
        }
    } else {
        if (g.a_sk != 1 || g.b_sk != 1 || g.splits != 1 || (g.K % BK) != 0) return -3;
        if ((long)g.M * g.a_si * 2 >= (1L << 31) || (long)g.N * g.b_sj * 2 >= (1L << 31)) return -3;
        r = launch_kc_any(epi, g, s);
    }
    if (r) return r;
    if (kname) *kname = g_last_kernel;
    return hipGetLastError() == hipSuccess ? 0 : -2;
}

int launch_tr_probe(unsigned short* out, hipStream_t s) {
    MRGAN_LAUNCH(tr_probe_kernel, dim3(1), dim3(64), 0, s, out);
    return hipGetLastError() == hipSuccess ? 0 : -2;
}

}
```

mr_gan_amd/engine.py:

```python
import ctypes as C
import os

import numpy as np
import torch

_HERE = os.path.dirname(os.path.abspath(__file__))
LIB_PATH = os.path.join(_HERE, "lib", "libmrgan_hip.so")

F32, BF16, FP8 = 0, 1, 2
NET_G, NET_D = 0, 1
FLAG_SYNC_STATS, FLAG_FLAT_GRADS, FLAG_GRAPH, FLAG_GRAD_BF16, FLAG_GAUSS_NOISE = 1, 2, 4, 8, 16
NOISE_MODES = ('irwin-hall', 'gaussian')
D_GEN, D_MAIN, D_ADAM = 0, 1, 2
G_GEN, G_FEAT, G_BWD, G_TAIL, G_ADAM = 0, 1, 2, 3, 4
TUNE_CHAIN, TUNE_KC_CFG, TUNE_KS_GROUP, TUNE_PAIR_GEN, TUNE_HEAD_MFMA = 0, 1, 4, 5, 6
REGION_BN_STATS, REGION_FM_MOMENTS, REGION_BN_BWD, REGION_GRAD_D, REGION_GRAD_G, REGION_WORKSPACE = range(6)
REGION_GRAD_D_BF16, REGION_GRAD_G_BF16, REGION_TAIL_D, REGION_TAIL_G = 6, 7, 8, 9

EXPORTS = [
    "mrgan_default_config", "mrgan_workspace_bytes", "mrgan_create", "mrgan_destroy", "mrgan_last_error",
    "mrgan_num_tensors", "mrgan_tensor_shape", "mrgan_set_weights", "mrgan_get_weights", "mrgan_get_slot",
    "mrgan_set_slot", "mrgan_get_iterations", "mrgan_set_iterations", "mrgan_disc_step", "mrgan_gen_step",
    "mrgan_train_pair", "mrgan_sup_step", "mrgan_fp8_calibration", "mrgan_logmel", "mrgan_logmel_frames", "mrgan_region", "mrgan_eval_error", "mrgan_predict_logits", "mrgan_read_metrics",
    "mrgan_pair_hint", "mrgan_set_tuning", "mrgan_debug_noise", "mrgan_debug_tr_probe", "mrgan_debug_gemm_launch", "mrgan_profile_begin", "mrgan_profile_end", "mrgan_debug_ablate", "mrgan_debug_gemm_time", "mrgan_debug_buffer", "mrgan_debug_gemm_fp8",
    "mrgan_debug_quant8", "mrgan_debug_fp8_update_scales",
    "mrgan_select_model", "mrgan_sup_step_group",
]
MAX_MODELS = 16
PROF_NAME_LEN = 96


class Config(C.Structure):
    _fields_ = [
        ("d_in", C.c_int32), ("batch", C.c_int32), ("noise_size", C.c_int32),
        ("g_hidden", C.c_int32 * 2), ("d_hidden", C.c_int32 * 5),
        ("num_classes", C.c_int32), ("dtype", C.c_int32),
        ("sigma", C.c_float * 5),
        ("lr", C.c_float), ("beta1", C.c_float), ("beta2", C.c_float), ("adam_eps", C.c_float),
        ("bn_eps", C.c_float), ("unlabeled_weight", C.c_float),
        ("seed", C.c_uint64),
        ("rank", C.c_int32), ("world", C.c_int32), ("flags", C.c_int32), ("models", C.c_int32),
    ]


class DiscArgs(C.Structure):
    _fields_ = [
        ("x_lab", C.c_void_p), ("idx_lab", C.c_void_p), ("labels", C.c_void_p),
        ("x_unl", C.c_void_p), ("idx_unl", C.c_void_p), ("z", C.c_void_p),
        ("ld_x_lab", C.c_int64), ("ld_x_unl", C.c_int64),
        ("stream_mode", C.c_int32), ("reserved", C.c_int32),
    ]


class GenArgs(C.Structure):
    _fields_ = [
        ("x_unl", C.c_void_p), ("idx_unl", C.c_void_p), ("z", C.c_void_p),
        ("ld_x_unl", C.c_int64),
        ("stream_mode", C.c_int32), ("reserved", C.c_int32),
    ]


class SupArgs(C.Structure):
    _fields_ = [
        ("x", C.c_void_p), ("idx", C.c_void_p), ("labels", C.c_void_p),
        ("ld_x", C.c_int64),
        ("stream_mode", C.c_int32), ("rows_valid", C.c_int32),
    ]


class SupGroupArgs(C.Structure):
    _fields_ = [
        ("x", C.c_void_p), ("idx", C.c_void_p), ("labels", C.c_void_p),
        ("ld_x", C.c_int64),
        ("x_model_stride", C.c_int64), ("idx_model_stride", C.c_int64), ("labels_model_stride", C.c_int64),
        ("stream_mode", C.c_int32), ("rows_valid", C.c_int32),
    ]


_lib = None


def load_library(path=None):
    global _lib, LIB_PATH
    if _lib is not None:
        return _lib
    if path is not None:
        LIB_PATH = path
    if not os.path.exists(LIB_PATH):
        raise RuntimeError(
            "libmrgan_hip.so not found at %s -- build it with `python -c 'import __graft_entry__ as g; g.build()'` "
            "(there is no CPU fallback for the training path)" % LIB_PATH)
    lib = C.CDLL(LIB_PATH)
    lib.mrgan_last_error.restype = C.c_char_p
    for name in EXPORTS:
        if name != "mrgan_last_error":
            getattr(lib, name).restype = C.c_int
    _lib = lib
    return lib


class MrganError(RuntimeError):
    pass


def _check(rc):
    if rc != 0:
        raise MrganError("libmrgan_hip error %d: %s" % (rc, load_library().mrgan_last_error().decode()))


def default_config(d_in, batch):
    cfg = Config()
    _check(load_library().mrgan_default_config(C.byref(cfg), int(d_in), int(batch)))
    return cfg


def noise_flags(noise):
    if noise not in NOISE_MODES:
        raise ValueError("noise must be one of %s, got %r" % (NOISE_MODES, noise))
    return FLAG_GAUSS_NOISE if noise == 'gaussian' else 0


def _ptr(t):
    return C.c_void_p(t.data_ptr()) if t is not None else None


def _stream():
    return C.c_void_p(torch.cuda.current_stream().cuda_stream)


def _f32(t, dev):
    if isinstance(t, np.ndarray):
        t = torch.from_numpy(np.ascontiguousarray(t, dtype=np.float32))
    return t.to(device=dev, dtype=torch.float32).contiguous()


def exchange_regions(region, grad_dtype, which):
    if grad_dtype == 'bf16' and which in (REGION_GRAD_D, REGION_GRAD_G):
        d = which == REGION_GRAD_D
        return (region(REGION_GRAD_D_BF16 if d else REGION_GRAD_G_BF16), region(REGION_TAIL_D if d else REGION_TAIL_G))
    return (region(which),)


class Engine(object):

    def __init__(self, cfg, device="cuda:0"):
        if not torch.cuda.is_available():
            raise RuntimeError("mr_gan_amd needs a HIP device; there is no CPU path")
        self.lib = load_library()
        self.cfg = cfg
        self.device = torch.device(device)
        torch.cuda.set_device(self.device)
        nbytes = C.c_size_t()
        _check(self.lib.mrgan_workspace_bytes(C.byref(cfg), C.byref(nbytes)))
        self.workspace = torch.empty(nbytes.value + 512, dtype=torch.uint8, device=self.device)
        base = self.workspace.data_ptr()
        self._ws_off = (-base) % 256
        self.handle = C.c_void_p()
        _check(self.lib.mrgan_create(C.byref(cfg), C.c_void_p(base + self._ws_off), C.c_size_t(nbytes.value), _stream(),
                                     C.byref(self.handle)))
        self._keep = []

    def close(self):
        if getattr(self, "handle", None) is not None and self.handle:
            torch.cuda.synchronize(self.device)
            self.lib.mrgan_destroy(self.handle)
            self.handle = None

    def __del__(self):
        try:
            self.close()
        except Exception:
            pass

    def num_tensors(self, net):
        n = C.c_int()
        _check(self.lib.mrgan_num_tensors(self.handle, net, C.byref(n)))
        return n.value

    def tensor_shape(self, net, idx):
        r, c = C.c_int(), C.c_int()
        _check(self.lib.mrgan_tensor_shape(self.handle, net, idx, C.byref(r), C.byref(c)))
        return r.value, c.value

    def set_weights(self, net, tensors):
        for i, t in enumerate(tensors):
            r, c = self.tensor_shape(net, i)
            t = _f32(t, self.device)
            if t.numel() != r * c:
                raise ValueError("tensor %d of net %d: expected %d x %d, got %s" % (i, net, r, c, tuple(t.shape)))
            _check(self.lib.mrgan_set_weights(self.handle, net, i, _ptr(t), _stream()))
            self._keep.append(t)
        torch.cuda.current_stream().synchronize()
        self._keep = []

    def _fetch(self, net, fn, *extra):
        out = []
        for i in range(self.num_tensors(net)):
            r, c = self.tensor_shape(net, i)
            t = torch.empty(r * c, dtype=torch.float32, device=self.device)
            _check(fn(self.handle, net, i, *extra, _ptr(t), _stream()))
            full = self.full_shape(net, i)
            out.append(t.cpu().numpy().reshape(full))
        return out

    def full_shape(self, net, idx):
        r, c = self.tensor_shape(net, idx)
        is_matrix = (net == NET_D and idx % 2 == 0) or (net == NET_G and idx in (0, 4, 6))
        return (r, c) if is_matrix else (c,)

    def get_weights(self, net):
        return self._fetch(net, self.lib.mrgan_get_weights)

    def get_slot(self, net, which):
        return self._fetch(net, self.lib.mrgan_get_slot, which)

    def set_slot(self, net, which, tensors):
        for i, t in enumerate(tensors):
            t = _f32(t, self.device)
            _check(self.lib.mrgan_set_slot(self.handle, net, i, which, _ptr(t), _stream()))
            self._keep.append(t)
        torch.cuda.current_stream().synchronize()
        self._keep = []

    def get_iterations(self):
        it = C.c_uint32()
        _check(self.lib.mrgan_get_iterations(self.handle, _stream(), C.byref(it)))
        return it.value

    def set_iterations(self, iterations, batch_counter=0):
        _check(self.lib.mrgan_set_iterations(self.handle, C.c_uint32(iterations), C.c_uint32(batch_counter), _stream()))

    @staticmethod
    def disc_args(x_lab, labels, x_unl, z=None, idx_lab=None, idx_unl=None, stream_mode=0):
        a = DiscArgs()
        a.x_lab, a.idx_lab, a.labels = _ptr(x_lab), _ptr(idx_lab), _ptr(labels)
        a.x_unl, a.idx_unl, a.z = _ptr(x_unl), _ptr(idx_unl), _ptr(z)
        a.ld_x_lab, a.ld_x_unl = x_lab.stride(0), x_unl.stride(0)
        a.stream_mode = stream_mode
        a._refs = (x_lab, labels, x_unl, z, idx_lab, idx_unl)
        return a

    @staticmethod
    def gen_args(x_unl, z=None, idx_unl=None, stream_mode=0):
        a = GenArgs()
        a.x_unl, a.idx_unl, a.z = _ptr(x_unl), _ptr(idx_unl), _ptr(z)
        a.ld_x_unl = x_unl.stride(0)
        a.stream_mode = stream_mode
        a._refs = (x_unl, z, idx_unl)
        return a

    def disc_step(self, args, first=0, last=-1, want_outputs=True):
        out = (C.c_float * 3)()
        _check(self.lib.mrgan_disc_step(self.handle, C.byref(args), first, last, out if want_outputs else None, _stream()))
        return tuple(out) if want_outputs else None

    def gen_step(self, args, first=0, last=-1, want_outputs=True):
        out = (C.c_float * 1)()
        _check(self.lib.mrgan_gen_step(self.handle, C.byref(args), first, last, out if want_outputs else None, _stream()))
        return out[0] if want_outputs else None

    @staticmethod
    def sup_args(x, labels, idx=None, stream_mode=0, rows_valid=0):
        a = SupArgs()
        a.x, a.idx, a.labels = _ptr(x), _ptr(idx), _ptr(labels)
        a.ld_x = x.stride(0)
        a.stream_mode = stream_mode
        a.rows_valid = rows_valid
        a._refs = (x, labels, idx)
        return a

    def sup_step(self, args, want_outputs=True):
        out = (C.c_float * 2)()
        _check(self.lib.mrgan_sup_step(self.handle, C.byref(args), out if want_outputs else None, _stream()))
        return tuple(out) if want_outputs else None

    @property
    def models(self):
        return max(1, int(self.cfg.models))

    def select_model(self, model):
        _check(self.lib.mrgan_select_model(self.handle, int(model)))

    @staticmethod
    def sup_group_args(x, labels, idx=None, stream_mode=0, rows_valid=0, x_model_stride=None, idx_model_stride=None,
                       labels_model_stride=None):
        a = SupGroupArgs()
        a.x, a.idx, a.labels = _ptr(x), _ptr(idx), _ptr(labels)
        a.ld_x = x.stride(-2)
        a.x_model_stride = (x.stride(0) if x.dim() == 3 else 0) if x_model_stride is None else x_model_stride
        a.idx_model_stride = (idx.stride(0) if idx is not None and idx.dim() == 2 else 0) if idx_model_stride is None else idx_model_stride
        a.labels_model_stride = (labels.stride(0) if labels.dim() == 2 else 0) if labels_model_stride is None else labels_model_stride
        a.stream_mode, a.rows_valid = stream_mode, rows_valid
        a._refs = (x, labels, idx)
        return a

    def sup_step_group(self, args, want_outputs=True):
        out = (C.c_float * (2 * MAX_MODELS))()
        _check(self.lib.mrgan_sup_step_group(self.handle, C.byref(args), out if want_outputs else None, _stream()))
        return [(out[2 * m], out[2 * m + 1]) for m in range(self.models)] if want_outputs else None

    FP8_DRY_PASSES = 5
    FP8_CAL_QUERY, FP8_CAL_BEGIN, FP8_CAL_END_PASS, FP8_CAL_DONE = 0, 1, 2, 3

    def fp8_calibration(self, kind, action):
        rc = self.lib.mrgan_fp8_calibration(self.handle, int(kind), int(action), _stream())
        if rc < 0:
            _check(rc)
        return rc

    def train_pair(self, dargs, gargs):
        _check(self.lib.mrgan_train_pair(self.handle, C.byref(dargs), C.byref(gargs), _stream()))

    def set_tuning(self, knob, value):
        _check(self.lib.mrgan_set_tuning(self.handle, int(knob), int(value)))

    def pair_hint(self, on=True):
        _check(self.lib.mrgan_pair_hint(self.handle, 1 if on else 0))

    def eval_error(self, x, labels, idx=None):
        err = C.c_float()
        _check(self.lib.mrgan_eval_error(self.handle, _ptr(x), _ptr(idx), C.c_int64(x.stride(0)), _ptr(labels),
                                         C.c_int64(labels.numel() if idx is None else idx.numel()), C.byref(err), _stream()))
        return err.value

    def predict_logits(self, x, idx=None):
        n = x.shape[0] if idx is None else idx.numel()
        out = torch.empty((n, self.cfg.num_classes), dtype=torch.float32, device=self.device)
        _check(self.lib.mrgan_predict_logits(self.handle, _ptr(x), _ptr(idx), C.c_int64(x.stride(0)), C.c_int64(n), _ptr(out),
                                             _stream()))
        return out

    def read_metrics(self, reset=True):
        out = (C.c_float * 8)()
        _check(self.lib.mrgan_read_metrics(self.handle, out, 1 if reset else 0, _stream()))
        return list(out)

    def profile_begin(self):
        _check(self.lib.mrgan_profile_begin(self.handle))

    def profile_end(self, max_kernels=64):
        names = C.create_string_buffer(max_kernels * PROF_NAME_LEN)
        ms, cnt = (C.c_float * max_kernels)(), (C.c_int32 * max_kernels)()
        fl, by, n = (C.c_double * max_kernels)(), (C.c_double * max_kernels)(), C.c_int()
        _check(self.lib.mrgan_profile_end(self.handle, _stream(), max_kernels, names, ms, cnt, fl, by, C.byref(n)))
        out = {}
        for i in range(n.value):
            name = names.raw[i * PROF_NAME_LEN:(i + 1) * PROF_NAME_LEN].split(b"\0")[0].decode()
            if name != "(start)":
                out[name] = (ms[i], cnt[i], fl[i], by[i])
        return out

    def region(self, which):
        p, n = C.c_void_p(), C.c_size_t()
        _check(self.lib.mrgan_region(self.handle, which, C.byref(p), C.byref(n)))
        off = p.value - self.workspace.data_ptr()
        return self.workspace[off:off + n.value].view(torch.bfloat16 if which in (REGION_GRAD_D_BF16, REGION_GRAD_G_BF16) else torch.float32)

    @property
    def grad_dtype(self):
        return 'bf16' if self.cfg.flags & FLAG_GRAD_BF16 else None

    def exchange_regions(self, which):
        return exchange_regions(self.region, self.grad_dtype, which)

    def debug_ablate(self, bits):
        _check(self.lib.mrgan_debug_ablate(self.handle, int(bits)))

    def debug_buffer(self, kind, l, nseg=3):
        p, rows, ld, es = C.c_void_p(), C.c_int(), C.c_int(), C.c_int()
        _check(self.lib.mrgan_debug_buffer(self.handle, kind, l, C.byref(p), C.byref(rows), C.byref(ld), C.byref(es)))
        off = p.value - self.workspace.data_ptr()
        n = nseg * rows.value * ld.value * es.value
        raw = self.workspace[off:off + n]
        t = raw.view(torch.bfloat16 if es.value == 2 else torch.float32)
        return t.reshape(nseg, rows.value, ld.value).float().clone()

    def debug_noise(self, site, seg, step, rows, cols, row0=0):
        out = torch.empty((rows, cols), dtype=torch.float32, device=self.device)
        _check(self.lib.mrgan_debug_noise(self.handle, site, seg, step, row0, rows, cols, _ptr(out), _stream()))
        return out


class DebugGemmDesc(C.Structure):
    _fields_ = [
        ("dtype", C.c_int32), ("op", C.c_int32), ("m", C.c_int32), ("n", C.c_int32), ("k", C.c_int32),
        ("nbatch", C.c_int32), ("splits", C.c_int32), ("kchunk", C.c_int32), ("kc_cfg", C.c_int32), ("tune_bits", C.c_int32),
        ("seg_stride", C.c_int32), ("seg_rows", C.c_int32),
        ("a", C.c_void_p), ("a_bs", C.c_int64), ("a_si", C.c_int64), ("a_sk", C.c_int64),
        ("b", C.c_void_p), ("b_bs", C.c_int64), ("b_sk", C.c_int64), ("b_sj", C.c_int64),
        ("act", C.c_int32), ("n_valid", C.c_int32), ("bias", C.c_void_p),
        ("out", C.c_void_p), ("out_bs", C.c_int64), ("ldo", C.c_int32),
        ("sigma", C.c_float), ("site", C.c_uint32), ("seg0", C.c_uint32), ("seg_step", C.c_int32),
        ("iter_step", C.c_uint32), ("row0", C.c_uint32), ("iter", C.c_uint32), ("seed", C.c_uint64),
        ("mask", C.c_void_p), ("mask_bs", C.c_int64), ("ldm", C.c_int32),
        ("h", C.c_void_p), ("h_bs", C.c_int64), ("ldh", C.c_int32),
        ("cs_mode", C.c_int32), ("cs1", C.c_void_p), ("cs2", C.c_void_p), ("ldcs", C.c_int32),
        ("bn_mu", C.c_void_p), ("bn_rstd", C.c_void_p),
        ("slab", C.c_void_p), ("slab_stride", C.c_int64),
        ("q8", C.c_void_p), ("q8_bs", C.c_int64), ("ldq8", C.c_int32),
        ("q8t", C.c_void_p), ("q8t_bs", C.c_int64), ("ldq8t", C.c_int32),
        ("slot_a", C.c_void_p), ("slot_b", C.c_void_p), ("slot_o", C.c_void_p),
        ("gauss", C.c_int32),
    ]


class DebugFold(C.Structure):
    _fields_ = [("src", C.c_void_p), ("dst", C.c_void_p), ("stride", C.c_int64), ("nsrc", C.c_int32), ("n", C.c_int32),
                ("ngroups", C.c_int32)]


def debug_gemm_desc(**kw):
    d = DebugGemmDesc()
    d.kc_cfg, d.nbatch, d.splits = -1, 1, 1
    d._refs = []
    for name, v in kw.items():
        if isinstance(v, torch.Tensor):
            d._refs.append(v)
            v = v.data_ptr()
        setattr(d, name, v)
    return d


def debug_gemm_launch(descs, grouped=False, fold=None):
    if isinstance(descs, DebugGemmDesc):
        descs = [descs]
    arr = (DebugGemmDesc * len(descs))(*descs)
    name = C.create_string_buffer(PROF_NAME_LEN)
    f = None
    if fold is not None:
        src, dst, stride, nsrc, n, ngroups = fold
        f = DebugFold(src.data_ptr(), dst.data_ptr(), stride, nsrc, n, ngroups)
    rc = load_library().mrgan_debug_gemm_launch(arr, len(descs), 1 if grouped else 0, C.byref(f) if f is not None else None,
                                                name, PROF_NAME_LEN, _stream())
    if rc not in (0, 1, -1, -3):
        _check(rc)
    return rc, name.value.decode()


def debug_gemm(dtype, op, a, b, bias=None, act=0, splits=1):
    td = torch.bfloat16 if dtype == BF16 else torch.float32
    m = a.shape[0]
    k, n = (a.shape[1], b.shape[1]) if op == 2 else b.shape
    if n % 64 or k % 64:
        raise ValueError("debug_gemm: n and k must be multiples of 64")
    a, b = a.to(td).contiguous(), b.to(td).contiguous()
    if op == 0:
        wt = dtype == BF16
        out = torch.zeros((m, n), dtype=td, device=a.device)
        d = debug_gemm_desc(dtype=dtype, op=0, m=m, n=n, k=k, a=a, a_si=k, a_sk=1, b=b.t().contiguous() if wt else b,
                            b_sk=1 if wt else n, b_sj=k if wt else 1, act=act, n_valid=n, bias=bias, out=out, ldo=n)
    elif op == 1:
        out = torch.zeros((m, k), dtype=td, device=a.device)
        d = debug_gemm_desc(dtype=dtype, op=1, m=m, n=k, k=n, a=a, a_si=n, a_sk=1, b=b, b_sk=1, b_sj=n, n_valid=k, out=out, ldo=k)
    else:
        splits = max(1, splits)
        out = torch.zeros((splits, k, n), dtype=torch.float32, device=a.device)
        d = debug_gemm_desc(dtype=dtype, op=2, m=k, n=n, k=m, splits=splits, kchunk=-(-(-(-m // splits)) // 64) * 64,
                            a=a, a_si=1, a_sk=k, b=b, b_sk=n, b_sj=1, slab=out, slab_stride=k * n, ldo=n)
    _check(debug_gemm_launch(d)[0])
    for s in range(1, splits if op == 2 else 0):
        out[0] += out[s]
    return out[0] if op == 2 else out.float()


def fp8_slots(rows, device="cuda:0"):
    return torch.from_numpy(np.array(rows, dtype=np.float32).reshape(-1, 4).view(np.int32)).to(device)


def fp8_slots_read(slots):
    w = slots.cpu().numpy()
    return w[:, 0].view(np.uint32).copy(), w[:, 1:].copy().view(np.float32)


def debug_quant8(src, src_bs, ld, rows, cols, nb, prow, slot, fmt, dst=None, dst_bs=0, ldd=0, dstt=None, dstt_bs=0, lddt=0):
    rc = load_library().mrgan_debug_quant8(_ptr(src), C.c_int64(src_bs), int(ld), int(rows), int(cols), int(nb), int(prow), _ptr(dst),
                                           C.c_int64(dst_bs), int(ldd), _ptr(dstt), C.c_int64(dstt_bs), int(lddt), _ptr(slot), int(fmt),
                                           _stream())
    if rc not in (0, -1, -3):
        _check(rc)
    return rc


def debug_fp8_update_scales(slots):
    _check(load_library().mrgan_debug_fp8_update_scales(_ptr(slots), int(slots.shape[0]), _stream()))


def debug_tr_probe(device="cuda:0"):
    out = torch.zeros(1024, dtype=torch.int16, device=device)
    _check(load_library().mrgan_debug_tr_probe(_ptr(out), _stream()))
    return out.cpu().numpy().astype(np.uint16).reshape(2, 64, 8)


def debug_gemm_time(op, m, n, k, nbatch=1, splits=1, reps=50, ablate=0, kc_cfg=-1):
    us = C.c_float()
    _check(load_library().mrgan_debug_gemm_time(op, m, n, k, nbatch, splits, reps, ablate, kc_cfg, C.byref(us)))
    return us.value


def debug_gemm_fp8(a, b, bias=None, act=0, scale_a=1.0, scale_b=1.0, reps=0, kc_cfg=-1):
    m, k = a.shape
    n = b.shape[1]
    out = torch.empty((m, n), dtype=torch.float32, device=a.device)
    us = C.c_float()
    _check(load_library().mrgan_debug_gemm_fp8(m, n, k, _ptr(a), _ptr(b), _ptr(bias), act, C.c_float(scale_a), C.c_float(scale_b), _ptr(out),
                                               reps, C.byref(us), int(kc_cfg), _stream()))
    return out, us.value
```

Before: 2616 steps/s.

## Precompute GEMM tile-decode heads and load compact kernargs in one burst

Adds a 128-byte precomputed GemmHead to the GEMM arguments, holding tile counts, byte strides and multiply-shift divisors, plus XCD-interleaved and patch tile orderings. Kernels read it with a single scalar burst load of the kernel-argument segment. The split-K weight-gradient group kernel now takes compact 64-byte per-problem descriptors instead of full GemmArgs copies. The aim is to cut per-block setup latency (kernarg fetch, integer divisions) and to improve tile locality across XCDs, at the cost of more complex planning code and new debug entry points for checking tile order.

```diff
diff --git a/include/mrgan_debug.h b/include/mrgan_debug.h
--- a/include/mrgan_debug.h
+++ b/include/mrgan_debug.h
@@ -42,6 +42,21 @@
 int mrgan_debug_gemm_launch(const mrgan_debug_gemm_desc* d, int count, int grouped, const mrgan_debug_fold* fold,
                             char* kname, int kname_len, mrgan_stream stream);
 
+typedef struct mrgan_debug_plan {
+    int32_t cfg, bm, bn, grid;
+    int32_t ntm, ntn, tpb, ntiles, nk;
+    uint32_t flags;
+    int32_t a_rsb, b_rsb, ext_a, ext_b;
+    int64_t a_bsb, b_bsb;
+    uint8_t head[128];
+} mrgan_debug_plan;
+int mrgan_debug_gemm_plan(int op, int m, int n, int k, int nbatch, int models, int kc_cfg, mrgan_debug_plan* out);
+int mrgan_debug_gemm_tile(const mrgan_debug_plan* plan, int first, int count, int32_t* out);
+int mrgan_debug_dw_group_plan(int count, const int32_t* m, const int32_t* n, const int32_t* k, const int32_t* splits, int fold_n,
+                              int fold_ngroups, int32_t* blk_end, int32_t* total);
+int mrgan_debug_dw_group_block(int count, const int32_t* m, const int32_t* n, const int32_t* k, const int32_t* splits, int fold_n,
+                               int fold_ngroups, int first, int nblocks, int32_t* out);
+
 int mrgan_debug_gemm_fp8(int m, int n, int k, const float* a_dev, const float* b_dev, const float* bias_dev, int act, float scale_a,
                          float scale_b, float* out_dev, int reps, float* avg_us, int kc_cfg, mrgan_stream stream);
 
diff --git a/mr_gan_amd/csrc/engine_debug.hip b/mr_gan_amd/csrc/engine_debug.hip
--- a/mr_gan_amd/csrc/engine_debug.hip
+++ b/mr_gan_amd/csrc/engine_debug.hip
@@ -111,10 +111,10 @@
     if (stamps) {
         std::vector<unsigned long long> hs(4096 * 12);
         hipMemcpy(hs.data(), stamps, hs.size() * 8, hipMemcpyDeviceToHost);
-        double tot[10] = {0, 0, 0, 0, 0, 0, 0, 0, 0, 0}; int nb = 0;
-        for (int b = 0; b < 4096; ++b) if (hs[b * 12 + 2]) { ++nb; for (int i = 0; i < 10; ++i) tot[i] += (double)hs[b * 12 + i]; }
-        if (nb) fprintf(stderr, "  stamps (kcycles per block, %d blocks): setup %.1f | fill %.1f | mainloop %.1f | barrier %.1f | epilogue %.1f (math+staging %.1f, barrier %.1f, copy-out %.1f, column sums %.1f) | tail-barrier %.1f\n",
-                        nb, tot[0] / nb / 1e3, tot[1] / nb / 1e3, tot[2] / nb / 1e3, tot[3] / nb / 1e3, tot[4] / nb / 1e3, tot[6] / nb / 1e3, tot[7] / nb / 1e3, tot[8] / nb / 1e3,
+        double tot[11] = {0, 0, 0, 0, 0, 0, 0, 0, 0, 0, 0}; int nb = 0;
+        for (int b = 0; b < 4096; ++b) if (hs[b * 12 + 2]) { ++nb; for (int i = 0; i < 11; ++i) tot[i] += (double)hs[b * 12 + i]; }
+        if (nb) fprintf(stderr, "  stamps (kcycles per block, %d blocks): setup %.1f (of which until the head of the arguments arrived %.1f) | fill %.1f | mainloop %.1f | barrier %.1f | epilogue %.1f (math+staging %.1f, barrier %.1f, copy-out %.1f, column sums %.1f) | tail-barrier %.1f\n",
+                        nb, tot[0] / nb / 1e3, tot[10] / nb / 1e3, tot[1] / nb / 1e3, tot[2] / nb / 1e3, tot[3] / nb / 1e3, tot[4] / nb / 1e3, tot[6] / nb / 1e3, tot[7] / nb / 1e3, tot[8] / nb / 1e3,
                         tot[9] / nb / 1e3, tot[5] / nb / 1e3);
         hipFree(stamps);
     }
@@ -240,6 +240,80 @@
     return 0;
 }
 
+int mrgan_debug_gemm_plan(int op, int m, int n, int k, int nbatch, int models, int kc_cfg, mrgan_debug_plan* out) {
+    if (!out || (op != 0 && op != 1) || m < 1 || n < 1 || k < 1 || nbatch < 1 || models < 1 || (n % 64) || (k % 64)) return fail(-1, "debug_gemm_plan: bad argument");
+    if (!kc_cfg_supported(kc_cfg)) return fail(-1, "debug_gemm_plan: kc_cfg %d is not a block tile", kc_cfg);
+    static uint16_t some_mask;
+    GemmArgs g = gemm_args(m, n, k, nbatch, 64);
+    g.a_bs = (long)m * k; g.a_si = k; g.a_sk = 1; g.b_sj = k; g.b_sk = 1;
+    g.e.act = ACT_RELU; g.e.n_valid = n; g.e.tune_kc_cfg = kc_cfg;
+    if (op == 1) g.e.mask = &some_mask;
+    g = gemm_group(g, models, (long)n * k * 2);
+    GemmHead hd;
+    if (const int r = gemm_bf16_kc_plan(op == 0 ? EPI_FWD : EPI_DX, g, &hd, &out->cfg, &out->bm, &out->bn, &out->grid)) return fail(r, "debug_gemm_plan: refused (%d)", r);
+    out->ntm = hd.ntm; out->ntn = hd.ntn; out->tpb = hd.tpb; out->ntiles = hd.ntiles; out->nk = hd.nk; out->flags = hd.flags;
+    out->a_rsb = hd.a_rsb; out->b_rsb = hd.b_rsb; out->ext_a = hd.ext_a; out->ext_b = hd.ext_b; out->a_bsb = hd.a_bsb; out->b_bsb = hd.b_bsb;
+    static_assert(sizeof out->head == sizeof hd, "the plan carries the head");
+    memcpy(out->head, &hd, sizeof hd);
+    return 0;
+}
+
+int mrgan_debug_gemm_tile(const mrgan_debug_plan* plan, int first, int count, int32_t* out) {
+    if (!plan || !out || first < 0 || count < 0 || first + count > plan->ntiles) return fail(-1, "debug_gemm_tile: bad argument");
+    GemmHead hd;
+    memcpy(&hd, plan->head, sizeof hd);
+    for (int i = 0; i < count; ++i) {
+        const GemmTile t = gemm_tile_decode(hd, first + i);
+        out[4 * i] = t.model; out[4 * i + 1] = t.seg; out[4 * i + 2] = t.tile_m; out[4 * i + 3] = t.tile_n;
+    }
+    return 0;
+}
+
+static int debug_dw_group(int count, const int32_t* m, const int32_t* n, const int32_t* k, const int32_t* splits, int fold_n, int fold_ngroups,
+                          KsGroup& grp, int& total) {
+    if (count < 1 || count > KS_GROUP_MAX || !m || !n || !k || !splits || fold_n < 0 || (fold_n > 0 && fold_ngroups < 1)) return fail(-1, "debug_dw_group: bad argument");
+    GemmArgs gs[KS_GROUP_MAX];
+    for (int i = 0; i < count; ++i) {
+        if (m[i] < 1 || n[i] < 1 || k[i] < 1 || splits[i] < 1) return fail(-1, "debug_dw_group: empty problem");
+        gs[i] = gemm_dw_args(m[i], n[i], k[i], splits[i], gemm_dw_kchunk(k[i], splits[i]), 0, 0, nullptr, m[i], nullptr, n[i], false, nullptr);
+    }
+    FoldJob fj;
+    memset(&fj, 0, sizeof fj);
+    fj.n = fold_n; fj.ngroups = fold_ngroups; fj.stride = fold_n; fj.nsrc = fold_ngroups;
+    return gemm_bf16_dw_group_plan(gs, count, fold_n > 0 ? &fj : nullptr, &grp, &total) ? 0 : 1;
+}
+
+int mrgan_debug_dw_group_plan(int count, const int32_t* m, const int32_t* n, const int32_t* k, const int32_t* splits, int fold_n,
+                              int fold_ngroups, int32_t* blk_end, int32_t* total) {
+    if (!blk_end || !total) return fail(-1, "null argument");
+    KsGroup grp;
+    int tot = 0;
+    if (const int r = debug_dw_group(count, m, n, k, splits, fold_n, fold_ngroups, grp, tot)) return r;
+    for (int i = 0; i < count; ++i) blk_end[i] = grp.hd.blk_end[i];
+    *total = tot;
+    return 0;
+}
+
+int mrgan_debug_dw_group_block(int count, const int32_t* m, const int32_t* n, const int32_t* k, const int32_t* splits, int fold_n,
+                               int fold_ngroups, int first, int nblocks, int32_t* out) {
+    if (!out) return fail(-1, "null argument");
+    KsGroup grp;
+    int tot = 0;
+    if (const int r = debug_dw_group(count, m, n, k, splits, fold_n, fold_ngroups, grp, tot)) return r;
+    if (first < 0 || nblocks < 0 || first + nblocks > tot) return fail(-1, "debug_dw_group_block: blocks outside the grid");
+    for (int j = 0; j < nblocks; ++j) {
+        const int block = first + j;
+        int32_t* o = out + 4 * j;
+        int b0 = 0, blocks = 0;
+        const int i = ks_group_problem(grp.hd, block, b0, blocks);
+        o[0] = i; o[1] = o[2] = o[3] = 0;
+        if (i >= count) { o[1] = block - b0; continue; }
+        const KsTile t = ks_tile_decode(grp.d[i], block - b0, blocks);
+        o[1] = t.split; o[2] = t.tile_m; o[3] = t.tile_n;
+    }
+    return 0;
+}
+
 int mrgan_debug_gemm_launch(const mrgan_debug_gemm_desc* d, int count, int grouped, const mrgan_debug_fold* fold,
                             char* kname, int kname_len, mrgan_stream stream) {
     if (!d || count < 1) return fail(-1, "null argument");
diff --git a/mr_gan_amd/csrc/gemm.h b/mr_gan_amd/csrc/gemm.h
--- a/mr_gan_amd/csrc/gemm.h
+++ b/mr_gan_amd/csrc/gemm.h
@@ -40,7 +40,78 @@
     uint32_t model_mul;
 };
 
+struct DivU32 { uint32_t mul, shift; };
+__host__ __device__ inline DivU32 div_u32_make(uint32_t d) {
+    uint32_t l = 0;
+    while ((1ull << l) < d) ++l;
+    const unsigned long long p = 1ull << (31 + l);
+    DivU32 r;
+    r.mul = (uint32_t)((p + d - 1) / d); r.shift = 31 + l;
+    return r;
+}
+__host__ __device__ __forceinline__ int div_u32(DivU32 m, int n) { return (int)(((unsigned long long)(uint32_t)n * m.mul) >> m.shift); }
+__host__ __device__ __forceinline__ int div_u31(uint32_t mul, int n) { return (int)(((unsigned long long)(uint32_t)n * mul) >> 31); }
+
+enum { PLAN_XCD = 1, PLAN_PATCH = 2 };
+struct GemmHead {
+    const void* A; const void* B;
+    long a_bsb, b_bsb;
+    long model_stride;
+    int a_rsb, b_rsb;
+    int ext_a, ext_b;
+    int ntm, ntn, tpb, ntiles;
+    int nk;
+    uint32_t flags;
+    uint32_t model_mul; int segs;
+    DivU32 div_tpb, div_row;
+    int pad_[6];
+};
+static_assert(sizeof(GemmHead) == 128, "the head is two 64-byte lines");
+
+struct TileIdx { int outer, tile_m, tile_n; };
+__host__ __device__ __forceinline__ TileIdx tile_decode(int tl, int ntiles, int tpb, int ntn, uint32_t flags, DivU32 div_tpb, DivU32 div_row) {
+    const int tidx = (flags & PLAN_XCD) ? (tl & 7) * (ntiles >> 3) + (tl >> 3) : tl;
+    TileIdx t;
+    t.outer = div_u32(div_tpb, tidx);
+    const int rem = tidx - t.outer * tpb;
+    if (flags & PLAN_PATCH) {
+        const int pl = (int)(flags >> 8), grp = div_u32(div_row, rem), in = rem - grp * (ntn << pl);
+        t.tile_m = (grp << pl) + (in & ((1 << pl) - 1)); t.tile_n = in >> pl;
+    } else { t.tile_m = div_u32(div_row, rem); t.tile_n = rem - t.tile_m * ntn; }
+    return t;
+}
+struct GemmTile { int model, seg, tile_m, tile_n; };
+__host__ __device__ __forceinline__ GemmTile gemm_tile_decode(const GemmHead& h, int tl) {
+    const TileIdx t = tile_decode(tl, h.ntiles, h.tpb, h.ntn, h.flags, h.div_tpb, h.div_row);
+    GemmTile r;
+    r.model = (int)(((uint32_t)t.outer * h.model_mul) >> 16); r.seg = t.outer - r.model * h.segs;
+    r.tile_m = t.tile_m; r.tile_n = t.tile_n;
+    return r;
+}
+
+typedef __attribute__((ext_vector_type(16))) uint32_t u32x16_s;
+template <typename H>
+__device__ __forceinline__ H kernarg_burst(const void* at = nullptr ) {
+    static_assert(sizeof(H) == 64 || sizeof(H) == 128, "whole lines");
+    typedef const __attribute__((address_space(4))) u32x16_s* lines_t;
+    lines_t kp = at ? (lines_t)at : (lines_t)__builtin_amdgcn_kernarg_segment_ptr();
+    struct Lines { u32x16_s w[sizeof(H) / 64]; } l;
+#pragma unroll
+    for (int i = 0; i < (int)(sizeof(H) / 64); ++i) l.w[i] = kp[i];
+    if constexpr (sizeof(H) == 128) asm volatile("" : "+s"(l.w[0]), "+s"(l.w[1]));
+    else asm volatile("" : "+s"(l.w[0]));
+    return __builtin_bit_cast(H, l);
+}
+template <typename T>
+__device__ __forceinline__ const T& kernarg_tail() {
+    typedef const __attribute__((address_space(4))) T* p4_t;
+    p4_t p = (p4_t)__builtin_amdgcn_kernarg_segment_ptr();
+    asm volatile("" : "+s"(p));
+    return *(const T*)p;
+}
+
 struct GemmArgs {
+    GemmHead hd;
     int M, N, K;
     int nbatch, splits;
     int kchunk;
@@ -82,12 +153,13 @@
 
 template <typename T, int EPI, int MR, int NR, int VAR>
 __device__ __forceinline__ void epilogue_prefetch(EpiPrefetch<MR, NR>& pf, const GemmArgs& g, int batch , int model,
-                                                  int row_blk, int col_blk, int wm, int wn, int lane) {
+                                                  int row_blk, int col_blk, int wm, int wn, int lane,
+                                                  bool iter_known = false, uint32_t iter = 0u ) {
     const Epi& e = g.e;
     const int lc = lane & 31, lh = lane >> 5;
     const int act = (VAR & 64) ? e.act : (VAR & 3);
-    pf.iter = 0u;
-    if constexpr (EPI == EPI_FWD && ((VAR & VAR_DYN) || (VAR & VAR_NOISE))) { if (e.st) pf.iter = e.st->iter; }
+    pf.iter = iter;
+    if constexpr (EPI == EPI_FWD && ((VAR & VAR_DYN) || (VAR & VAR_NOISE))) { if (!iter_known && e.st) pf.iter = e.st->iter; }
 #pragma unroll
     for (int ni = 0; ni < NR; ++ni) {
         const int col = col_blk + (wn * NR + ni) * 32 + lc;
@@ -399,15 +471,55 @@
 }
 constexpr int KS_GROUP_MAX = 6;
 struct FoldJob { const float* src; float* dst; long stride; int nsrc, n, ngroups, blocks_x; long model_stride; };
+struct KsDesc {
+    const void* A; const void* B; float* slab;
+    uint32_t slab_stride; int ldo;
+    int M, N, K, kchunk;
+    int a_sk, b_sk;
+    uint32_t mul_tpb, mul_row;
+};
+static_assert(sizeof(KsDesc) == 64, "one line per problem");
+__host__ __device__ __forceinline__ uint32_t ks_order_flags(int ntm, int ntn, int blocks) {
+    return ((blocks & 7) == 0 ? PLAN_XCD : 0u) | (((ntm & 7) == 0 && ntn >= 16) ? (PLAN_PATCH | (3u << 8)) : 0u);
+}
+struct KsTile { int split, tile_m, tile_n; };
+__host__ __device__ __forceinline__ KsTile ks_tile_decode(const KsDesc& d, int bid, int blocks) {
+    const int ntn = (d.N + 127) >> 7, ntm = (d.M + 127) >> 7;
+    const DivU32 dt = {d.mul_tpb, 31}, dr = {d.mul_row, 31};
+    const TileIdx t = tile_decode(bid, blocks, ntn * ntm, ntn, ks_order_flags(ntm, ntn, blocks), dt, dr);
+    KsTile r;
+    r.split = t.outer; r.tile_m = t.tile_m; r.tile_n = t.tile_n;
+    return r;
+}
+struct KsSingle { KsDesc d; long model_stride; int ablate; int blocks ; int pad_[12]; };
+static_assert(sizeof(KsSingle) == 128, "two lines");
+struct KsGroupHead {
+    int n;
+    int ablate;
+    int blk_end[KS_GROUP_MAX];
+    int pad_[8];
+};
+static_assert(sizeof(KsGroupHead) == 64, "one line");
 struct KsGroup {
-    int n;
-    int blk_end[KS_GROUP_MAX];
+    KsGroupHead hd;
     FoldJob fold;
-    GemmArgs g[KS_GROUP_MAX];
-};
+    long model_stride[KS_GROUP_MAX];
+    alignas(64) KsDesc d[KS_GROUP_MAX];
+};
+__host__ __device__ __forceinline__ int ks_group_problem(const KsGroupHead& h, int b, int& b0, int& blocks) {
+    int i = 0, end = h.blk_end[0];
+    b0 = 0;
+#pragma unroll
+    for (int j = 0; j < KS_GROUP_MAX; ++j)
+        if (j < h.n && b >= h.blk_end[j]) { i = j + 1; b0 = h.blk_end[j]; end = j + 1 < KS_GROUP_MAX ? h.blk_end[j + 1] : b0; }
+    blocks = end - b0;
+    return i;
+}
 
 int launch_gemm_f32(int epi, const GemmArgs& g, hipStream_t s, const char** kname = nullptr);
 int launch_gemm_bf16(int epi, const GemmArgs& g, hipStream_t s, const char** kname = nullptr);
+int gemm_bf16_kc_plan(int epi, const GemmArgs& g, GemmHead* hd, int* cfg, int* bm, int* bn, int* grid);
+bool gemm_bf16_dw_group_plan(const GemmArgs* gs, int n, const FoldJob* fold, KsGroup* grp, int* total);
 int launch_gemm_fp8(int epi, const GemmArgs& g, hipStream_t s, const char** kname = nullptr);
 int launch_to_fp8(const float* src, long ld_src, unsigned char* dst, long ld_dst, int rows, int cols, int prow, int pcol, float scale,
                   int transpose, hipStream_t s);
@@ -468,6 +580,35 @@
 }
 inline int gemm_model_batches(const GemmArgs& g) { return g.e.segs > 0 ? g.e.segs : g.nbatch; }
 inline int gemm_models(const GemmArgs& g) { return g.e.segs > 0 ? g.nbatch / g.e.segs : 1; }
+inline GemmHead gemm_head(const GemmArgs& g, int BM, int BNT, int bk, int elem_bytes, int patch_rows_log2, bool patch) {
+    GemmHead h;
+    memset(&h, 0, sizeof h);
+    h.A = g.A; h.B = g.B;
+    h.a_bsb = g.a_bs * elem_bytes; h.b_bsb = g.b_bs * elem_bytes; h.model_stride = g.e.model_stride;
+    h.a_rsb = (int)(g.a_si * elem_bytes); h.b_rsb = (int)(g.b_sj * elem_bytes);
+    h.ext_a = (int)((long)g.M * g.a_si * elem_bytes); h.ext_b = (int)((long)g.N * g.b_sj * elem_bytes);
+    h.ntm = ceil_div(g.M, BM); h.ntn = ceil_div(g.N, BNT); h.tpb = h.ntm * h.ntn; h.ntiles = h.tpb * g.nbatch;
+    h.nk = (g.e.ablate & 4) ? 0 : g.K / bk;
+    patch = patch && (h.ntm & ((1 << patch_rows_log2) - 1)) == 0;
+    h.flags = ((h.ntiles & 7) == 0 ? PLAN_XCD : 0u) | (patch ? (PLAN_PATCH | ((uint32_t)patch_rows_log2 << 8)) : 0u);
+    h.model_mul = g.e.model_mul; h.segs = g.e.segs;
+    h.div_tpb = div_u32_make((uint32_t)h.tpb);
+    h.div_row = div_u32_make((uint32_t)(patch ? h.ntn << patch_rows_log2 : h.ntn));
+    return h;
+}
+inline bool ks_plan(const GemmArgs& g, KsDesc& d, int& blocks) {
+    const int ntn = ceil_div(g.N, 128), ntm = ceil_div(g.M, 128);
+    blocks = ntn * ntm * g.splits;
+    const uint32_t drow = ((ks_order_flags(ntm, ntn, blocks) & PLAN_PATCH) ? 8u : 1u) * (uint32_t)ntn;
+    if ((long)blocks * (ntn * ntm) >= (1L << 31) || (long)blocks * drow >= (1L << 31)) return false;
+    if (g.e.slab_stride < 0 || g.e.slab_stride >= (1L << 32) || g.a_sk >= (1L << 31) || g.b_sk >= (1L << 31)) return false;
+    memset(&d, 0, sizeof d);
+    d.A = g.A; d.B = g.B; d.slab = g.e.slab; d.slab_stride = (uint32_t)g.e.slab_stride; d.ldo = g.e.ldo;
+    d.M = g.M; d.N = g.N; d.K = g.K; d.kchunk = g.kchunk; d.a_sk = (int)g.a_sk; d.b_sk = (int)g.b_sk;
+    d.mul_tpb = (uint32_t)(((1ull << 31) + (uint32_t)(ntn * ntm) - 1) / (uint32_t)(ntn * ntm));
+    d.mul_row = (uint32_t)(((1ull << 31) + drow - 1) / drow);
+    return true;
+}
 inline long mask_pitch(int seg_rows, int ldm) { return (long)(seg_rows / 32) * ldm * 2; }
 
 inline int epi_variant(int epi, const Epi& e) {
diff --git a/mr_gan_amd/csrc/gemm_bf16.hip b/mr_gan_amd/csrc/gemm_bf16.hip
--- a/mr_gan_amd/csrc/gemm_bf16.hip
+++ b/mr_gan_amd/csrc/gemm_bf16.hip
@@ -12,63 +12,95 @@
 constexpr int KS_PITCH = 320;
 constexpr int KS_TILE_BYTES = 64 * KS_PITCH;
 
+inline GemmHead kc_head(const GemmArgs& g, int BM, int BNT) {
+    return gemm_head(g, BM, BNT, BK, 2, 2, ceil_div(g.N, BNT) >= 8 && g.K >= 2048);
+}
+
 #ifdef MRGAN_STAMPS
-struct KcStamps { unsigned long long acc[6], prev, epi[5]; };
-#define KC_STAMPS_PARAM , KcStamps& stamps_
-#define KC_STAMPS_ARG , stamps_
-#else
-#define KC_STAMPS_PARAM
-#define KC_STAMPS_ARG
+struct KcStamps { unsigned long long acc[6], prev, epi[5], head; };
 #endif
+template <int EPI, int BM, int BNT, int WM, int NS, int VAR>
+constexpr int kc_lds_bytes() {
+    constexpr int STAGE = BM * 128 + BNT * 128, OUT = BM * BNT * 2 + 4 * WM * BNT * 4;
+    return (NS * STAGE > OUT ? NS * STAGE : OUT) + ((EPI == EPI_DX && (VAR & VAR_ACT_MASK) != ACT_RELU) ? BM * BNT * 2 : 0);
+}
+template <int LDS, int NW>
+constexpr int kc_waves_per_simd() {
+    constexpr int blocks = (160 * 1024) / LDS > 1 ? (160 * 1024) / LDS : 1, w = blocks * NW / 4;
+    return w > 8 ? 8 : w < 1 ? 1 : w;
+}
 template <int EPI, int BM, int BNT, int WM, int WN, int NS, int VAR>
-__device__ __forceinline__ void kc_tile(const GemmArgs& g, const int batch , const int model, const int tile_m, const int tile_n, char* lds KC_STAMPS_PARAM) {
+__global__ __launch_bounds__(64 * WM * WN) __attribute__((amdgpu_waves_per_eu(kc_waves_per_simd<kc_lds_bytes<EPI, BM, BNT, WM, NS, VAR>(), WM * WN>())))
+void gemm_bf16_kc_kernel(const GemmArgs g_) {
+    extern __shared__ __attribute__((aligned(16))) char lds[];
     constexpr int NW = WM * WN;
     constexpr int MR = BM / WM / 32, NR = BNT / WN / 32;
     constexpr int A_BYTES = BM * 128, B_BYTES = BNT * 128, STAGE = A_BYTES + B_BYTES;
     constexpr int A_INSTR = BM / 8 / NW, B_INSTR = BNT / 8 / NW;
     static_assert(MR >= 1 && NR >= 1 && A_INSTR >= 1 && B_INSTR >= 1 && BM % (8 * NW) == 0 && BNT % (8 * NW) == 0, "tile/wave layout");
+#ifdef MRGAN_STAMPS
+    KcStamps stamps_ = {{0, 0, 0, 0, 0, 0}, __builtin_amdgcn_s_memtime(), {0, 0, 0, 0, 0}, 0};
+    asm volatile("s_waitcnt lgkmcnt(0)" ::: "memory");
+#endif
+    const GemmHead hd = kernarg_burst<GemmHead>();
+#ifdef MRGAN_STAMPS
+    stamps_.head = __builtin_amdgcn_s_memtime() - stamps_.prev;
+#define STAMP(i) do { const unsigned long long n_ = __builtin_amdgcn_s_memtime(); stamps_.acc[i] += n_ - stamps_.prev; stamps_.prev = n_; } while (0)
+#else
+#define STAMP(i)
+#endif
     const int t = threadIdx.x, lane = t & 63;
     const int wave = __builtin_amdgcn_readfirstlane(t >> 6);
     const int wm = wave / WN, wn = wave % WN;
     const int lrow = lane >> 3, lp = lane & 7;
     const int lr = lane & 31, lh = lane >> 5;
-    const int nk = (g.e.ablate & 4) ? 0 : g.K / BK;
-#ifdef MRGAN_STAMPS
-#define STAMP(i) do { const unsigned long long n_ = __builtin_amdgcn_s_memtime(); stamps_.acc[i] += n_ - stamps_.prev; stamps_.prev = n_; } while (0)
-#else
-#define STAMP(i)
-#endif
-    {
-        const int row_blk = tile_m * BM, col_blk = tile_n * BNT;
-
-        const __bf16* Ab = model_ptr((const __bf16*)g.A, g.e, model) + (long)batch * g.a_bs;
-        const __bf16* Bb = model_ptr((const __bf16*)g.B, g.e, model) + (long)batch * g.b_bs;
-        const __amdgpu_buffer_rsrc_t rsA = __builtin_amdgcn_make_buffer_rsrc((void*)Ab, 0, (int)((long)g.M * g.a_si * 2), 0x00020000);
-        const __amdgpu_buffer_rsrc_t rsB = __builtin_amdgcn_make_buffer_rsrc((void*)Bb, 0, (int)((long)g.N * g.b_sj * 2), 0x00020000);
-        int voffA[A_INSTR], voffB[B_INSTR];
+    const int nk = hd.nk;
+
+    GemmTile tile;
+    __amdgpu_buffer_rsrc_t rsA, rsB;
+    int voffA[A_INSTR], voffB[B_INSTR];
+    auto place = [&](int tl) {
+        tile = gemm_tile_decode(hd, tl);
+        const long moff = (long)tile.model * hd.model_stride;
+        rsA = __builtin_amdgcn_make_buffer_rsrc((void*)((const char*)hd.A + moff + (long)tile.seg * hd.a_bsb), 0, hd.ext_a, 0x00020000);
+        rsB = __builtin_amdgcn_make_buffer_rsrc((void*)((const char*)hd.B + moff + (long)tile.seg * hd.b_bsb), 0, hd.ext_b, 0x00020000);
 #pragma unroll
         for (int i = 0; i < A_INSTR; ++i) {
             const int R = (wave * A_INSTR + i) * 8 + lrow;
-            voffA[i] = (int)(((long)(row_blk + R) * g.a_si + ((lp ^ ((R >> 1) & 7)) << 3)) * 2);
+            voffA[i] = (int)((uint32_t)(tile.tile_m * BM + R) * (uint32_t)hd.a_rsb + (uint32_t)((lp ^ ((R >> 1) & 7)) << 4));
         }
 #pragma unroll
         for (int i = 0; i < B_INSTR; ++i) {
             const int R = (wave * B_INSTR + i) * 8 + lrow;
-            voffB[i] = (int)(((long)(col_blk + R) * g.b_sj + ((lp ^ ((R >> 1) & 7)) << 3)) * 2);
-        }
-        auto issue = [&](int k0, int buf) {
-            char* a_dst = lds + buf * STAGE + wave * A_INSTR * 1024;
-            char* b_dst = lds + buf * STAGE + A_BYTES + wave * B_INSTR * 1024;
-#pragma unroll
-            for (int i = 0; i < A_INSTR; ++i) glds16(rsA, a_dst + i * 1024, voffA[i], k0 * 2);
-#pragma unroll
-            for (int i = 0; i < B_INSTR; ++i) glds16(rsB, b_dst + i * 1024, voffB[i], k0 * 2);
-        };
-
+            voffB[i] = (int)((uint32_t)(tile.tile_n * BNT + R) * (uint32_t)hd.b_rsb + (uint32_t)((lp ^ ((R >> 1) & 7)) << 4));
+        }
+    };
+    auto issue = [&](int k0, int buf) {
+        char* a_dst = lds + buf * STAGE + wave * A_INSTR * 1024;
+        char* b_dst = lds + buf * STAGE + A_BYTES + wave * B_INSTR * 1024;
+#pragma unroll
+        for (int i = 0; i < A_INSTR; ++i) glds16(rsA, a_dst + i * 1024, voffA[i], k0 * 2);
+#pragma unroll
+        for (int i = 0; i < B_INSTR; ++i) glds16(rsB, b_dst + i * 1024, voffB[i], k0 * 2);
+    };
+    auto fill = [&]() {
 #pragma unroll
         for (int p = 0; p < NS - 1; ++p)
             if (p < nk) issue(p * BK, p);
-
+    };
+
+    int tl = blockIdx.x;
+    if (tl >= hd.ntiles) return;
+    place(tl);
+    fill();
+    __builtin_amdgcn_sched_barrier(0);
+    const GemmArgs& g = kernarg_tail<GemmArgs>();
+    uint32_t iter = 0u;
+    if constexpr (EPI == EPI_FWD && (VAR & VAR_NOISE) != 0) { if (g.e.st) iter = g.e.st->iter; }
+
+    for (;;) {
+        const int batch = tile.seg, model = tile.model, tile_m = tile.tile_m;
+        const int row_blk = tile_m * BM, col_blk = tile.tile_n * BNT;
 
         const __bf16* htile = nullptr;
         if constexpr (EPI == EPI_DX && (VAR & VAR_ACT_MASK) != ACT_RELU) {
@@ -99,7 +131,7 @@
                 for (int r = 0; r < 16; ++r) acc[i][j][r] = 0.f;
 
         EpiPrefetch<MR, NR> pf;
-        epilogue_prefetch<__bf16, EPI, MR, NR, VAR>(pf, g, batch, model, row_blk, col_blk, wm, wn, lane);
+        epilogue_prefetch<__bf16, EPI, MR, NR, VAR>(pf, g, batch, model, row_blk, col_blk, wm, wn, lane, true, iter);
 
 #define KC_FRAG_A(As, mi, ks) *(const bf16x8*)(As + kc_off((wm * MR + mi) * 32 + lr, (ks) * 2 + lh))
 #define KC_FRAG_B(Bs, ni, ks) *(const bf16x8*)(Bs + kc_off((wn * NR + ni) * 32 + lr, (ks) * 2 + lh))
@@ -118,34 +150,18 @@
         STAMP(4);
         __syncthreads();
         STAMP(5);
+        tl += gridDim.x;
+        if (tl >= hd.ntiles) break;
+        place(tl);
+        fill();
     }
 #undef STAMP
-}
-
-template <int EPI, int BM, int BNT, int WM, int WN, int NS, int VAR>
-__global__ __launch_bounds__(64 * WM * WN) void gemm_bf16_kc_kernel(const GemmArgs g) {
-    extern __shared__ __attribute__((aligned(16))) char lds[];
-    const int ntn = (g.N + BNT - 1) / BNT, ntm = (g.M + BM - 1) / BM;
-    const int ntiles = ntn * ntm * g.nbatch;
-#ifdef MRGAN_STAMPS
-    KcStamps stamps_ = {{0, 0, 0, 0, 0, 0}, __builtin_amdgcn_s_memtime(), {0, 0, 0, 0, 0}};
-#endif
-    for (int tl = blockIdx.x; tl < ntiles; tl += gridDim.x) {
-        const int tidx = xcd_tile(tl, ntiles);
-        const int bidx = tidx / (ntn * ntm), rem = tidx - bidx * (ntn * ntm);
-        const int model = batch_model(g.e, bidx), batch = batch_segment(g.e, bidx, model);
-        int tile_m, tile_n;
-        if ((ntm & 3) == 0 && ntn >= 8 && g.K >= 2048) {
-            const int grp = rem / (4 * ntn), in = rem - grp * (4 * ntn);
-            tile_m = grp * 4 + (in & 3); tile_n = in >> 2;
-        } else { tile_m = rem / ntn; tile_n = rem - tile_m * ntn; }
-        kc_tile<EPI, BM, BNT, WM, WN, NS, VAR>(g, batch, model, tile_m, tile_n, lds KC_STAMPS_ARG);
-    }
 #ifdef MRGAN_STAMPS
     if (g.e.slab && threadIdx.x == 0)
     {
         for (int i = 0; i < 6; ++i) ((unsigned long long*)g.e.slab)[(long)blockIdx.x * 12 + i] = stamps_.acc[i];
         for (int i = 0; i < 4; ++i) ((unsigned long long*)g.e.slab)[(long)blockIdx.x * 12 + 6 + i] = stamps_.epi[i];
+        ((unsigned long long*)g.e.slab)[(long)blockIdx.x * 12 + 10] = stamps_.head;
     }
 #endif
 }
@@ -158,11 +174,10 @@
                                     std::to_string(BNT) + ", " + std::to_string(WM) + ", " + std::to_string(WN) + ", " +
                                     std::to_string(NS) + ", " + std::to_string(VAR) + ">";
     g_last_kernel = name.c_str();
-    constexpr int STAGE = BM * 128 + BNT * 128;
-    constexpr int OUT = BM * BNT * 2 + 4 * WM * BNT * 4;
-    constexpr int LDS = (NS * STAGE > OUT ? NS * STAGE : OUT) + ((EPI == EPI_DX && (VAR & VAR_ACT_MASK) != ACT_RELU) ? BM * BNT * 2 : 0);
-    const int tiles = ceil_div(g.M, BM) * ceil_div(g.N, BNT) * g.nbatch;
-    return launch_with_dyn_lds<gemm_bf16_kc_kernel<EPI, BM, BNT, WM, WN, NS, VAR>, LDS>(dim3(persistent_grid(tiles, LDS)), dim3(64 * WM * WN), s, g);
+    constexpr int LDS = kc_lds_bytes<EPI, BM, BNT, WM, NS, VAR>();
+    GemmArgs p = g;
+    p.hd = kc_head(g, BM, BNT);
+    return launch_with_dyn_lds<gemm_bf16_kc_kernel<EPI, BM, BNT, WM, WN, NS, VAR>, LDS>(dim3(persistent_grid(p.hd.ntiles, LDS)), dim3(64 * WM * WN), s, p);
 }
 
 __device__ __forceinline__ bf16x8 ks_frag_swz(const char* tile, int fb, int ks, int lane) {
@@ -177,7 +192,7 @@
 }
 
 template <int NS, int WM, int WN>
-__device__ __forceinline__ void ks_fast_body(const GemmArgs& g, const int bid, const int model ) {
+__device__ __forceinline__ void ks_fast_body(const KsDesc& d, const int bid, const int blocks, const long moff, const int ablate) {
     constexpr int NW = WM * WN;
     constexpr int MR = 128 / WM / 32, NR = 128 / WN / 32;
     constexpr int T_BYTES = 64 * 256, STAGE = 2 * T_BYTES;
@@ -188,50 +203,45 @@
     const int t = threadIdx.x, lane = t & 63;
     const int wave = __builtin_amdgcn_readfirstlane(t >> 6);
     const int wm = wave / WN, wn = wave % WN;
-    const int ntn = (g.N + 127) / 128, ntm = (g.M + 127) / 128;
-    const int tidx = xcd_tile(bid, ntn * ntm * g.splits);
-    const int split = tidx / (ntn * ntm), rem = tidx - split * (ntn * ntm);
-    int tile_m, tile_n;
-    if ((ntm & 7) == 0 && ntn >= 16) {
-        const int grp = rem / (8 * ntn), in = rem - grp * (8 * ntn);
-        tile_m = grp * 8 + (in & 7); tile_n = in >> 3;
-    } else { tile_m = rem / ntn; tile_n = rem - tile_m * ntn; }
-    const int row_blk = tile_m * 128, col_blk = tile_n * 128;
-    const int k_begin = split * g.kchunk;
-    const int k_end = (g.e.ablate & 4) ? k_begin : min(g.K, k_begin + g.kchunk);
-
-    const __amdgpu_buffer_rsrc_t rsA = __builtin_amdgcn_make_buffer_rsrc((void*)model_ptr(g.A, g.e, model), 0, (int)((long)g.K * g.a_sk * 2), 0x00020000);
-    const __amdgpu_buffer_rsrc_t rsB = __builtin_amdgcn_make_buffer_rsrc((void*)model_ptr(g.B, g.e, model), 0, (int)((long)g.K * g.b_sk * 2), 0x00020000);
+    const KsTile tile = ks_tile_decode(d, bid, blocks);
+    const int split = tile.split, tile_m = tile.tile_m;
+    const int row_blk = tile_m * 128, col_blk = tile.tile_n * 128;
+    const int k_begin = split * d.kchunk;
+    const int k_end = (ablate & 4) ? k_begin : min(d.K, k_begin + d.kchunk);
+
+    const __amdgpu_buffer_rsrc_t rsA = __builtin_amdgcn_make_buffer_rsrc((void*)((const char*)d.A + moff), 0, (int)((long)d.K * d.a_sk * 2), 0x00020000);
+    const __amdgpu_buffer_rsrc_t rsB = __builtin_amdgcn_make_buffer_rsrc((void*)((const char*)d.B + moff), 0, (int)((long)d.K * d.b_sk * 2), 0x00020000);
     const int lrow = lane >> 4, lp = lane & 15;
     int voffA[T_INSTR], voffB[T_INSTR];
 #pragma unroll
     for (int i = 0; i < T_INSTR; ++i) {
         const int kr = (wave * T_INSTR + i) * 4 + lrow;
         const int c = lp ^ ((kr & 3) << 2);
-        voffA[i] = (int)(((long)kr * g.a_sk + row_blk + c * 8) * 2);
-        voffB[i] = (int)(((long)kr * g.b_sk + col_blk + c * 8) * 2);
+        voffA[i] = (int)(((long)kr * d.a_sk + row_blk + c * 8) * 2);
+        voffB[i] = (int)(((long)kr * d.b_sk + col_blk + c * 8) * 2);
     }
     auto issue = [&](int k0, int buf) {
         char* a_dst = lds + buf * STAGE + wave * T_INSTR * 1024;
         char* b_dst = a_dst + T_BYTES;
 #pragma unroll
-        for (int i = 0; i < T_INSTR; ++i) glds16(rsA, a_dst + i * 1024, voffA[i], (int)((long)k0 * g.a_sk * 2));
-#pragma unroll
-        for (int i = 0; i < T_INSTR; ++i) glds16(rsB, b_dst + i * 1024, voffB[i], (int)((long)k0 * g.b_sk * 2));
+        for (int i = 0; i < T_INSTR; ++i) glds16(rsA, a_dst + i * 1024, voffA[i], (int)((long)k0 * d.a_sk * 2));
+#pragma unroll
+        for (int i = 0; i < T_INSTR; ++i) glds16(rsB, b_dst + i * 1024, voffB[i], (int)((long)k0 * d.b_sk * 2));
     };
-
-    f32x16 acc[MR][NR];
-#pragma unroll
-    for (int i = 0; i < MR; ++i)
-#pragma unroll
-        for (int j = 0; j < NR; ++j)
-#pragma unroll
-            for (int r = 0; r < 16; ++r) acc[i][j][r] = 0.f;
 
     const int nk = (k_end - k_begin + BK - 1) / BK;
 #pragma unroll
     for (int p = 0; p < NS - 1; ++p)
         if (p < nk) issue(k_begin + p * BK, p);
+
+    f32x16 acc[MR][NR];
+#pragma unroll
+    for (int i = 0; i < MR; ++i)
+#pragma unroll
+        for (int j = 0; j < NR; ++j)
+#pragma unroll
+            for (int r = 0; r < 16; ++r) acc[i][j][r] = 0.f;
+
 #define KS_FRAG_A(As, mi, ks) ks_frag_swz(As, (wm * MR + mi) * 32, ks, lane)
 #define KS_FRAG_B(Bs, ni, ks) ks_frag_swz(Bs, (wn * NR + ni) * 32, ks, lane)
 #define KS_NO_STAMP(i)
@@ -240,22 +250,38 @@
 #undef KS_FRAG_B
 #undef KS_NO_STAMP
     __syncthreads();
-    epilogue<__bf16, EPI_SLAB, MR, NR, WM>(acc, g, 0, model, split, tile_m, row_blk, col_blk, wm, wn, lane, (float*)lds, BN);
+    float* dst = (float*)((char*)d.slab + moff) + (long)split * d.slab_stride;
+    if (ablate & 2) { if (acc[0][0][0] == 12345.678f) dst[0] = 1.f; return; }
+    const int lc = lane & 31, lh = lane >> 5;
+#pragma unroll
+    for (int mi = 0; mi < MR; ++mi)
+#pragma unroll
+        for (int ni = 0; ni < NR; ++ni) {
+            const int col = col_blk + (wn * NR + ni) * 32 + lc;
+#pragma unroll
+            for (int r = 0; r < 16; ++r) {
+                const int row = row_blk + (wm * MR + mi) * 32 + acc_row(r, lh);
+                if (row < d.M && col < d.N) dst[(long)row * d.ldo + col] = acc[mi][ni][r];
+            }
+        }
 }
 
 template <int NS, int WM, int WN>
-__global__ __launch_bounds__(64 * WM * WN) void gemm_bf16_ks_fast_kernel(const GemmArgs g) {
-    ks_fast_body<NS, WM, WN>(g, blockIdx.x, blockIdx.y);
+__global__ __launch_bounds__(64 * WM * WN) void gemm_bf16_ks_fast_kernel(const KsSingle a_) {
+    const KsSingle a = kernarg_burst<KsSingle>();
+    ks_fast_body<NS, WM, WN>(a.d, blockIdx.x, a.blocks, (long)blockIdx.y * a.model_stride, a.ablate);
 }
 
 template <int NS, int WM, int WN>
 __global__ __launch_bounds__(64 * WM * WN) void gemm_bf16_ks_group_kernel(const KsGroup grp) {
-    const int ngemm = grp.blk_end[grp.n - 1];
-    if ((int)blockIdx.x >= ngemm) {
+    const KsGroupHead gh = kernarg_burst<KsGroupHead>();
+    int b0, blocks;
+    const int i = ks_group_problem(gh, (int)blockIdx.x, b0, blocks);
+    if (i >= gh.n) {
         const FoldJob& f = grp.fold;
         const float* fsrc = (const float*)((const char*)f.src + (long)blockIdx.y * f.model_stride);
         float* fdst = (float*)((char*)f.dst + (long)blockIdx.y * f.model_stride);
-        const int fb = (int)blockIdx.x - ngemm, gidx = fb / f.blocks_x;
+        const int fb = (int)blockIdx.x - b0, gidx = fb / f.blocks_x;
         const int i = (fb - gidx * f.blocks_x) * 256 + (int)threadIdx.x;
         if (threadIdx.x >= 256 || i >= f.n) return;
         float s0 = 0.f, s1 = 0.f, s2 = 0.f, s3 = 0.f;
@@ -268,11 +294,9 @@
         fdst[(long)gidx * f.stride + i] = (s0 + s1) + (s2 + s3);
         return;
     }
-    int i = 0, b0 = 0;
-#pragma unroll
-    for (int j = 0; j < KS_GROUP_MAX - 1; ++j)
-        if (j + 1 < grp.n && (int)blockIdx.x >= grp.blk_end[j]) { i = j + 1; b0 = grp.blk_end[j]; }
-    ks_fast_body<NS, WM, WN>(grp.g[i], (int)blockIdx.x - b0, blockIdx.y);
+    const KsDesc d = kernarg_burst<KsDesc>(&grp.d[i]);
+    const long moff = blockIdx.y ? (long)blockIdx.y * grp.model_stride[i] : 0L;
+    ks_fast_body<NS, WM, WN>(d, (int)blockIdx.x - b0, blocks, moff, gh.ablate);
 }
 
 template <int NS, int WM, int WN>
@@ -280,8 +304,13 @@
     static const std::string name = "gemm_bf16_ks_fast_kernel<" + std::to_string(NS) + ", " + std::to_string(WM) + ", " + std::to_string(WN) + ">";
     g_last_kernel = name.c_str();
     constexpr int STAGE = 2 * 64 * 256;
-    dim3 grid(ceil_div(g.N, 128) * ceil_div(g.M, 128) * g.splits, gemm_models(g));
-    return launch_with_dyn_lds<gemm_bf16_ks_fast_kernel<NS, WM, WN>, NS * STAGE>(grid, dim3(64 * WM * WN), s, g);
+    KsSingle a;
+    memset(&a, 0, sizeof a);
+    int blocks = 0;
+    if (!ks_plan(g, a.d, blocks)) return -3;
+    a.model_stride = g.e.model_stride; a.ablate = g.e.ablate; a.blocks = blocks;
+    dim3 grid(blocks, gemm_models(g));
+    return launch_with_dyn_lds<gemm_bf16_ks_fast_kernel<NS, WM, WN>, NS * STAGE>(grid, dim3(64 * WM * WN), s, a);
 }
 
 __device__ __forceinline__ bf16x8 ks_frag(const char* tile, int fb, int ks, int lane) {
@@ -383,8 +412,7 @@
 }
 }
 
-template <int EPI, int VAR>
-static int launch_kc_tile(const GemmArgs& g, hipStream_t s) {
+static int kc_pick_cfg(int EPI, bool h_tile, const GemmArgs& g) {
     int cfg = g.e.tune_kc_cfg;
     if (cfg < 0) {
         const int nbm = gemm_model_batches(g);
@@ -398,8 +426,17 @@
     }
     if (cfg >= 2 && cfg != 9 && (g.N % 128) != 0) cfg = 0;
     if (cfg == 3 && (g.N % 256) != 0) cfg = 1;
+    if (h_tile && cfg >= 2 && cfg != 9) cfg = 1;
+    return cfg;
+}
+static void kc_cfg_tile(int cfg, int& bm, int& bn) {
+    bm = cfg == 3 ? 256 : (cfg == 7 || cfg == 1) ? 128 : 64;
+    bn = cfg == 3 ? 256 : cfg == 9 ? 64 : 128;
+}
+template <int EPI, int VAR>
+static int launch_kc_tile(const GemmArgs& g, hipStream_t s) {
     constexpr bool H_TILE = EPI == EPI_DX && (VAR & VAR_ACT_MASK) != ACT_RELU;
-    if (H_TILE && cfg >= 2 && cfg != 9) cfg = 1;
+    const int cfg = kc_pick_cfg(EPI, H_TILE, g);
     if constexpr (!H_TILE) {
         if (cfg == 7) return launch_kc<EPI, 128, 128, 2, 4, 2, VAR>(g, s);
         if (cfg == 3) return launch_kc<EPI, 256, 256, 2, 4, 2, VAR>(g, s);
@@ -438,26 +475,35 @@
            (long)g.K * g.a_sk * 2 < (1L << 31) && (long)g.K * g.b_sk * 2 < (1L << 31);
 }
 
-int launch_gemm_bf16_dw_group(const GemmArgs* gs, int n, hipStream_t s, const char** kname, const FoldJob* fold) {
-    if (n < 1 || n > KS_GROUP_MAX) return 1;
-    if (gs[0].e.tune_bits & TUNE_BIT_NO_KS_GROUP) return 1;
-    KsGroup grp;
+bool gemm_bf16_dw_group_plan(const GemmArgs* gs, int n, const FoldJob* fold, KsGroup* out, int* total_blocks) {
+    if (n < 1 || n > KS_GROUP_MAX) return false;
+    if (gs[0].e.tune_bits & TUNE_BIT_NO_KS_GROUP) return false;
+    KsGroup& grp = *out;
     memset(&grp, 0, sizeof grp);
-    grp.n = n;
+    grp.hd.n = n; grp.hd.ablate = gs[0].e.ablate;
     int total = 0;
     const int models = gemm_models(gs[0]);
     for (int i = 0; i < n; ++i) {
-        if (!ks_dense_k(gs[i]) || gemm_models(gs[i]) != models) return 1;
-        const int blocks = ceil_div(gs[i].N, 128) * ceil_div(gs[i].M, 128) * gs[i].splits;
+        int blocks = 0;
+        if (!ks_dense_k(gs[i]) || gemm_models(gs[i]) != models || !ks_plan(gs[i], grp.d[i], blocks)) return false;
         total += blocks;
-        grp.blk_end[i] = total;
-        grp.g[i] = gs[i];
+        grp.hd.blk_end[i] = total;
+        grp.model_stride[i] = gs[i].e.model_stride;
     }
     if (fold && fold->n > 0) {
         grp.fold = *fold;
         grp.fold.blocks_x = ceil_div(fold->n, 256);
         total += grp.fold.blocks_x * fold->ngroups;
     }
+    *total_blocks = total;
+    return true;
+}
+
+int launch_gemm_bf16_dw_group(const GemmArgs* gs, int n, hipStream_t s, const char** kname, const FoldJob* fold) {
+    KsGroup grp;
+    int total = 0;
+    if (!gemm_bf16_dw_group_plan(gs, n, fold, &grp, &total)) return 1;
+    const int models = gemm_models(gs[0]);
     constexpr int STAGE = 2 * 64 * 256, LDS = 2 * STAGE;
     if (const int r = launch_with_dyn_lds<gemm_bf16_ks_group_kernel<2, 2, 4>, LDS>(dim3(total, models), dim3(512), s, grp)) return r;
     if (kname) *kname = "gemm_bf16_ks_group_kernel<2, 2, 4>";
@@ -485,6 +531,21 @@
     return hipGetLastError() == hipSuccess ? 0 : -2;
 }
 
+int gemm_bf16_kc_plan(int epi, const GemmArgs& g, GemmHead* hd, int* cfg, int* bm, int* bn, int* grid) {
+    if (epi != EPI_FWD && epi != EPI_DX) return -3;
+    const int var = epi_variant(epi, g.e);
+    if (var < 0) return -3;
+    const bool h_tile = epi == EPI_DX && (var & VAR_ACT_MASK) != ACT_RELU;
+    *cfg = kc_pick_cfg(epi, h_tile, g);
+    kc_cfg_tile(*cfg, *bm, *bn);
+    *hd = kc_head(g, *bm, *bn);
+    const int wm = 2, ns = (*cfg == 9 || *cfg == 0) ? 3 : 2;
+    const int stage = *bm * 128 + *bn * 128, out = *bm * *bn * 2 + 4 * wm * *bn * 4;
+    const int lds = std::max(ns * stage, out) + (h_tile ? *bm * *bn * 2 : 0);
+    *grid = persistent_grid(hd->ntiles, lds);
+    return 0;
+}
+
 int launch_tr_probe(unsigned short* out, hipStream_t s) {
     MRGAN_LAUNCH(tr_probe_kernel, dim3(1), dim3(64), 0, s, out);
     return hipGetLastError() == hipSuccess ? 0 : -2;
diff --git a/mr_gan_amd/engine.py b/mr_gan_amd/engine.py
--- a/mr_gan_amd/engine.py
+++ b/mr_gan_amd/engine.py
@@ -24,6 +24,7 @@
     "mrgan_train_pair", "mrgan_sup_step", "mrgan_fp8_calibration", "mrgan_logmel", "mrgan_logmel_frames", "mrgan_region", "mrgan_eval_error", "mrgan_predict_logits", "mrgan_read_metrics",
     "mrgan_pair_hint", "mrgan_set_tuning", "mrgan_debug_noise", "mrgan_debug_tr_probe", "mrgan_debug_gemm_launch", "mrgan_profile_begin", "mrgan_profile_end", "mrgan_debug_ablate", "mrgan_debug_gemm_time", "mrgan_debug_buffer", "mrgan_debug_gemm_fp8",
     "mrgan_debug_quant8", "mrgan_debug_fp8_update_scales",
+    "mrgan_debug_gemm_plan", "mrgan_debug_gemm_tile", "mrgan_debug_dw_group_plan", "mrgan_debug_dw_group_block",
     "mrgan_select_model", "mrgan_sup_step_group",
 ]
 MAX_MODELS = 16
@@ -435,6 +436,40 @@
     if rc not in (0, 1, -1, -3):
         _check(rc)
     return rc, name.value.decode()
+
+
+class DebugPlan(C.Structure):
+    _fields_ = [("cfg", C.c_int32), ("bm", C.c_int32), ("bn", C.c_int32), ("grid", C.c_int32),
+                ("ntm", C.c_int32), ("ntn", C.c_int32), ("tpb", C.c_int32), ("ntiles", C.c_int32), ("nk", C.c_int32),
+                ("flags", C.c_uint32), ("a_rsb", C.c_int32), ("b_rsb", C.c_int32), ("ext_a", C.c_int32), ("ext_b", C.c_int32),
+                ("a_bsb", C.c_int64), ("b_bsb", C.c_int64), ("head", C.c_uint8 * 128)]
+
+
+def debug_gemm_plan(op, m, n, k, nbatch=1, models=1, kc_cfg=-1):
+    p = DebugPlan()
+    _check(load_library().mrgan_debug_gemm_plan(op, m, n, k, nbatch, models, kc_cfg, C.byref(p)))
+    return p
+
+
+def debug_gemm_tiles(plan):
+    lib = load_library()
+    out = np.zeros((plan.ntiles, 4), dtype=np.int32)
+    _check(lib.mrgan_debug_gemm_tile(C.byref(plan), 0, plan.ntiles, out.ctypes.data_as(C.c_void_p)))
+    return out
+
+
+def debug_dw_group_plan(problems, fold_n=0, fold_ngroups=0):
+    lib = load_library()
+    cnt = len(problems)
+    cols = [(C.c_int32 * cnt)(*[p[i] for p in problems]) for i in range(4)]
+    blk_end, total = (C.c_int32 * cnt)(), C.c_int32()
+    rc = lib.mrgan_debug_dw_group_plan(cnt, *cols, fold_n, fold_ngroups, blk_end, C.byref(total))
+    if rc == 1:
+        return None
+    _check(rc)
+    out = np.zeros((total.value, 4), dtype=np.int32)
+    _check(lib.mrgan_debug_dw_group_block(cnt, *cols, fold_n, fold_ngroups, 0, total.value, out.ctypes.data_as(C.c_void_p)))
+    return list(blk_end), total.value, out
 
 
 def debug_gemm(dtype, op, a, b, bias=None, act=0, splits=1):
```

Result: no change. 2642 steps/s (median of 6 runs) (+1.0%).
